# oleg-savchenko/jax_nbody_emulator_with_dj

Hardware: AMD Instinct MI355X
Metric: voxels/sec (disp+vel) on 512^3 box, ndiv=4 (higher is better)
Workload: dtype f32-equivalent: f16x3 split MFMA (3 f16 MFMAs per product, f32 accumulate)

## Files before the change

### jax_nbody_emulator_with_dj_amd/csrc/nbe_engine.cpp

```cpp

#include "../../include/nbe.h"
#include "nbe_kernels.h"

#include <sched.h>

#include <cmath>
#include <cstdarg>
#include <cstdio>
#include <cstdlib>
#include <cstring>
#include <algorithm>
#include <atomic>
#include <chrono>
#include <condition_variable>
#include <deque>
#include <map>
#include <memory>
#include <mutex>
#include <string>
#include <thread>
#include <vector>

using namespace nbe;

// ... 70 lines not shown

struct ProfEntry { std::string name; double ms = 0; int64_t launches = 0; double flops = 0; };

struct Progress {
    struct Item { hipEvent_t ev; int done, total; };
    nbe_progress_cb cb; void* user; int device;
    std::thread th; std::mutex mu; std::condition_variable cv; std::deque<Item> q; bool stop = false;
    Progress(nbe_progress_cb cb_, void* user_, int dev) : cb(cb_), user(user_), device(dev) {
        th = std::thread([this] {
            (void)hipSetDevice(device);
            for (;;) {
                Item it;
                {
                    std::unique_lock<std::mutex> lk(mu);
                    cv.wait(lk, [this] { return stop || !q.empty(); });
                    if (q.empty()) return;
                    it = q.front(); q.pop_front();
                }
                (void)hipEventSynchronize(it.ev);
                (void)hipEventDestroy(it.ev);
                cb(it.done, it.total, user);
            }
        });
    }
    void post(hipStream_t s, int done, int total) {
        hipEvent_t ev;
        if (hipEventCreateWithFlags(&ev, hipEventDisableTiming) != hipSuccess) return;
        (void)hipEventRecord(ev, s);
        { std::lock_guard<std::mutex> lk(mu); q.push_back({ev, done, total}); }
        cv.notify_one();
    }
    ~Progress() {
        { std::lock_guard<std::mutex> lk(mu); stop = true; }
        cv.notify_one();
        if (th.joinable()) th.join();
    }
};

struct nbe_ctx {
    int device = 0;
    hipStream_t own_stream = nullptr, stream = nullptr;
    int in_chan = 3, out_chan = 3, mid = 64;
    float eps = 1e-8f;
    bool vel = true;
    bool have_weights = false, style = false, modulated = false;
    float mod_Om = NAN, mod_Dz = NAN;
    std::map<std::string, Layer> layers;
    Arena arena;
    char* ws = nullptr;
    int64_t ws_bytes = 0;
    bool dry = false;
    int slab = 0;
    int slab_forced = -1;
    bool pyx = false;
    bool pyx_allowed = true;
    bool pz = false;
    bool zx = false;
    int phase = 0;
    struct BrickIO { void *send_lo = nullptr, *send_hi = nullptr; const void *recv_lo = nullptr, *recv_hi = nullptr;
                     void *skip_send_lo = nullptr, *skip_send_hi = nullptr; const void *skip_recv_lo = nullptr, *skip_recv_hi = nullptr;
                     hipEvent_t skip_ready = nullptr; } bio;
    struct StreamState {
        bool valid = false;
        int stage = 0;
        Tensor skip0, td, tin, t, h, y1, cat1, t2;
        int D = 0, H = 0, W = 0, S = 0;
        std::vector<Arena::Blk> blks; int64_t high = 0;
        float Dz = 0.f, vel_fac = 0.f, act_scale = 1.f; const char* ws = nullptr;
    } sst;
    nbe_progress_cb prog_cb = nullptr; void* prog_user = nullptr; int prog_k = 0, prog_n = 1;
    Progress* prog = nullptr;
    int max_tile = 512;
    int prec = PREC_F32;
    bool gauge = false;
    bool gauge_active = false;
    bool fuse = false;
    bool novel_fuse = false;
    int64_t bp_size[3] = {0, 0, 0}; int bp_slab = 0; int64_t bp_need = 0;
    int plan_tiles = 0;
    double plan_short_gb = 0.0;
    int64_t plan_logged = 0;
    int* gauge_flag = nullptr;
    int* wino_flag = nullptr; bool wino_ok = false;
    float act_scale = 1.f;
    float bias_scale = 1.f;
    bool bias_dirty = true;
    float bias_max = 0.f;
    float preset_absmax = -1.f;
    bool input_finite = true;
    bool range_pending = false;
    unsigned* flags = nullptr;
    float* box_in = nullptr; int64_t box_in_bytes = 0;
    char* box_out = nullptr; int64_t box_out_bytes = 0;
    struct HostPipe {
        bool active = false, out_async = false;
        bool tiles = false;
        bool slabwise = false;
        int o1 = 0, o2 = 0;
        const float* hbox = nullptr;
        bool in_pinned = false;
        int C = 0, S0 = 0, S1 = 0, S2 = 0, o0 = 0;
        std::vector<char> up;
        int gz = 0;
        char *hdisp = nullptr, *hvel = nullptr;
        char *ddisp = nullptr, *dvel = nullptr;
        int esz = 4, O0 = 0, O1 = 0, O2 = 0;
        int nstage = 0;
    } pipe;
    bool last_piped = false;
    hipStream_t up_stream = nullptr, down_stream = nullptr;
    static constexpr int NSTAGE = 3;
    char* stage_buf[NSTAGE] = {nullptr, nullptr, nullptr}; int64_t stage_bytes = 0;
    hipEvent_t stage_free[NSTAGE] = {nullptr, nullptr, nullptr};
    hipEvent_t ev_up = nullptr, ev_down = nullptr;
    struct GraphKey {
        const void *box, *disp, *velo, *ws;
        int geo[18]; float f[3]; int epoch, flags;
        bool operator<(const GraphKey& o) const { return memcmp(this, &o, sizeof *this) < 0; }
    };
    struct GraphVal { hipGraphExec_t exec = nullptr; hipGraph_t graph = nullptr; int seen = 0; uint64_t used = 0; };
    std::map<GraphKey, GraphVal> graphs;
    uint64_t graph_clock = 0, graph_replays = 0;
    int epoch = 0;
    hipEvent_t ev_g0 = nullptr, ev_g1 = nullptr;
    struct Probe {
        bool on = false, tile = false;
        int p[3] = {0, 0, 0}, nout = 0;
        int o[3] = {0, 0, 0};
        struct Slot { std::string name; int C, n, nw, level; int64_t off; };
        std::vector<Slot> slots;
        unsigned* bits = nullptr; int64_t words = 0;
        unsigned* count = nullptr;
    } probe;
    bool prof = false;
    std::vector<ProfEntry> prof_entries;
    struct Pending { int entry; hipEvent_t a, b; };
    std::vector<Pending> pending;
    std::vector<hipEvent_t> ev_pool;
};

static double hyp2f1_series(double a, double b, double c, double z) {
    double term = 1.0, sum = 1.0;
    for (int n = 0; n < 200000; ++n) {
        term *= (a + n) * (b + n) / ((c + n) * (n + 1.0)) * z;
        sum += term;
        if (std::fabs(term) < 1e-17 * std::fabs(sum)) break;
    }
    return sum;
}
static double hyp2f1(double a, double b, double c, double x) {
    if (x < 0) return std::pow(1.0 - x, -a) * hyp2f1_series(a, c - b, c, x / (x - 1.0));
    return hyp2f1_series(a, b, c, x);
}
static const double A2 = 1.0, B2 = 1.0 / 3.0, C2 = 11.0 / 6.0;

extern "C" double nbe_growth_factor(double z, double Om) {
    const double a = 1.0 / (1.0 + z), OL = 1.0 - Om;
    return a * hyp2f1(A2, B2, C2, -OL * a * a * a / Om) / hyp2f1(A2, B2, C2, -OL / Om);
}
static double growth_rate(double z, double Om) {
    const double a = 1.0 / (1.0 + z), x = -(1.0 - Om) * a * a * a / Om;
    const double F = hyp2f1(A2, B2, C2, x);
    const double dF = (A2 * B2 / C2) * hyp2f1(A2 + 1, B2 + 1, C2 + 1, x);
    return 1.0 + 3.0 * x * dF / F;
}
extern "C" double nbe_vel_norm(double z, double Om) {
// ... 106 lines not shown
    if (p.dx) p.dx += sh;
    return p;
}
static void fill_halo(nbe_ctx* c, const Tensor& t) {
    if (t.pad > 0 && !c->dry) launch_fill_yx(t.p, t.pad, c->vel, c->stream);
}
static void tfree(nbe_ctx* c, Tensor& t) { if (t.off >= 0) c->arena.release(t.off); t.off = -1; }
static Tensor zview(const Tensor& t, int z0, int nz) {
    Tensor v = t;
    v.off = -1;
    const int64_t sh = (int64_t)z0 * t.p.H * t.p.W * 4;
    if (v.p.x) v.p.x += sh;
    if (v.p.dx) v.p.dx += sh;
    v.p.D = nz;
    v.org[0] += z0;
    return v;
}
static void org_conv(const Tensor& x, int nconv, int out[3]) {
    const int p = x.pad ? nconv : 0;
    out[0] = x.org[0]; out[1] = x.org[1] - p; out[2] = x.org[2] - p;
}
static void set_org(Tensor& t, int z, int y, int x) { t.org[0] = z; t.org[1] = y; t.org[2] = x; }

static void probe_act(nbe_ctx* c, const Layer& L, const Planes& out, int g0, const int org[3], int ez, int ey, int ex, bool periodic,
                      const int* zr = nullptr) {
    auto& P = c->probe;
    if (!P.on || !P.tile || c->dry) return;
    const std::string name = L.block + "/" + L.layer;
    for (size_t i = 0; i < P.slots.size(); ++i) {
        const auto& S = P.slots[i];
        if (S.name != name) continue;
        ProbeLaunch a;
        a.x = out.x; a.pstride = out.pstride; a.H = out.H; a.W = out.W; a.g0 = g0; a.prec = c->prec; a.C = S.C;
        a.ext[0] = ez; a.ext[1] = ey; a.ext[2] = ex;
        a.org[0] = org[0]; a.org[1] = org[1]; a.org[2] = org[2];
        a.per[0] = 0; a.per[1] = periodic ? ey : 0; a.per[2] = periodic ? ex : 0;
        a.zlo = zr ? zr[0] : 0; a.zhi = zr ? zr[1] : 0; a.zper = zr ? zr[2] : 0;
        for (int d = 0; d < 3; ++d) a.o[d] = P.o[d] >> S.level;
        a.n = S.n; a.nw = S.nw;
        if (a.zper <= 0 && (a.o[0] + S.n <= org[0] || a.o[0] >= org[0] + ez)) return;
        a.bits = P.bits + S.off; a.count = P.count + i;
        launch_probe_signs(a, c->stream);
        return;
    }
}

static int prof_entry(nbe_ctx* c, const std::string& name) {
    for (size_t i = 0; i < c->prof_entries.size(); ++i) if (c->prof_entries[i].name == name) return (int)i;
    c->prof_entries.push_back({name, 0, 0, 0});
    return (int)c->prof_entries.size() - 1;
}
static hipEvent_t get_event(nbe_ctx* c) {
    if (!c->ev_pool.empty()) { hipEvent_t e = c->ev_pool.back(); c->ev_pool.pop_back(); return e; }
    hipEvent_t e; (void)hipEventCreate(&e); return e;
}
static void prof_collect(nbe_ctx* c) {
    if (c->pending.empty()) return;
    (void)hipStreamSynchronize(c->stream);
    for (auto& p : c->pending) {
        float ms = 0;
        (void)hipEventElapsedTime(&ms, p.a, p.b);
        c->prof_entries[p.entry].ms += ms;
        c->ev_pool.push_back(p.a); c->ev_pool.push_back(p.b);
    }
    c->pending.clear();
}

static std::string conv_name(const PackedW& pw, bool vel, bool has_dx, bool g6 = false, bool up8 = false) {
    if (up8) return vel ? "up_h3<8 parities,vel,dx>" : "up_h3<8 parities,novel>";
    const char* m = pw.mode == MODE_FLAT3 ? "FLAT3" : pw.mode == MODE_FLAT1 ? "FLAT1" : "DOWN";
    if (pw.stem && !(vel && has_dx) && pw.mode == MODE_FLAT3) return vel ? "stem_h3<FLAT3,vel,nodx>" : "stem_h3<FLAT3,novel>";
    char b[96];
    if (g6 && prec_is_half(pw.prec)) snprintf(b, sizeof b, "%s<%s,vel,dx>", pw.prec == PREC_F16 ? "conv_h1g" : (pw.cout_t == 16 ? "conv_h3n" : "conv_h3g"), m);
    else if (g6) snprintf(b, sizeof b, "conv_mfma_g<%s,vel,dx,ni%d>", m, pw.ni);
    else if (prec_is_half(pw.prec))
        snprintf(b, sizeof b, "%s<%s,%s,%s>", pw.prec == PREC_F16 ? "conv_h1" : "conv_h3", m, vel ? "vel" : "novel", (vel && has_dx) ? "dx" : "nodx");
    else
        snprintf(b, sizeof b, "conv_mfma<%s,%s,%s,ni%d>", m, vel ? "vel" : "novel", (vel && has_dx) ? "dx" : "nodx", pw.ni);
    return b;
}

static bool wino_f16_layer(int prec, bool vel, int cin_pad) { return prec == PREC_F16 && vel && cin_pad % 32 == 0 && cin_pad / 32 <= 8; }
static bool wino_env_off() { return getenv("NBE_WINO") && atoi(getenv("NBE_WINO")) == 0; }
static bool up8_launch(const nbe_ctx* c, const Layer& L, bool has_dx) { return prec_is_half(c->prec) && (!c->vel || has_dx) && L.pw.cin_pad <= 64; }

static int run_conv(nbe_ctx* c, const Layer& L, const ConvLaunch& cl_in, bool has_dx) {
    if (c->dry) return 0;
    ConvLaunch cl = cl_in;
    const bool g6 = c->gauge_active && L.g6 && has_dx;
    const bool nov = !c->vel && c->prec == PREC_F16X3 && L.kind == 0 && L.pw.ww && c->wino_ok;
    if (c->gauge_active) { cl.gout = L.gout; cl.beta = g6 ? L.beta : nullptr; }
    if (cl.skw) {
        if (!((g6 || nov) && c->fuse && L.fskip)) return fail("internal error: fused skip requested for %s/%s", L.block.c_str(), L.layer.c_str());
        cl.bias = L.bias_f;
    }
    const PackedW& pw = (g6 && L.kind == 0 && L.pwn.w) ? L.pwn : L.pw;
    cl.wino = (g6 || nov) && c->wino_ok && &pw == &L.pw && pw.ww && (!cl.skw || cl.skw->ww) && (c->prec == PREC_F16 || !(cl.flags & F_RES)) &&
              (cl.Dv & 1) == 0 && cl.in_off == 0 && cl.osz == 1 && !wino_env_off();
    int pe = -1; hipEvent_t ea = nullptr, eb = nullptr;
    if (c->prof) {
        std::string pn = cl.wino ? std::string(c->prec == PREC_F16 ? "conv_h1w<FLAT3,vel,dx>" : c->vel ? "conv_h3w<FLAT3,vel,dx>" : "conv_h3w<FLAT3,novel>")
                                 : conv_name(pw, c->vel, has_dx, g6, cl.set < 0);
        static const bool per_layer = getenv("NBE_PROF_LAYERS") && atoi(getenv("NBE_PROF_LAYERS")) == 1;
        if (per_layer) pn += " " + L.block + "/" + L.layer;
        pe = prof_entry(c, pn);
        ea = get_event(c); eb = get_event(c);
        (void)hipEventRecord(ea, c->stream);
    }
    if (launch_conv(pw, cl, c->vel, has_dx, c->stream))
        return fail("internal error: no kernel for layer %s/%s (mode %d, gauged %d, input tangent %d, crop offset %ld, output stride %d)",
                    L.block.c_str(), L.layer.c_str(), L.pw.mode, (int)g6, (int)has_dx, (long)cl.in_off, cl.osz);
    if (c->prof) {
        (void)hipEventRecord(eb, c->stream);
        c->pending.push_back({pe, ea, eb});
        const double nout = (double)cl.Dv * cl.Hv * cl.Wv * (cl.set < 0 ? 8.0 : 1.0);
        const int taps = L.kind == 0 ? 27 : L.kind == 2 ? 8 : 1;
        const double gemms = c->vel ? ((has_dx && !g6) ? 3.0 : 2.0) : 1.0;
        c->prof_entries[pe].flops += 2.0 * nout * L.cout * L.cin * taps * gemms;
        if (cl.skw) c->prof_entries[pe].flops += 2.0 * nout * L.cout * L.fskip->cin * (!c->vel ? 1.0 : (cl.flags & F_SKIP_NODX) ? 2.0 : 3.0);
        c->prof_entries[pe].launches += 1;
        if (c->pending.size() > 4096) prof_collect(c);
    }
    return 0;
}

static const Layer* find_layer(nbe_ctx* c, const char* block, const char* layer) {
    auto it = c->layers.find(std::string(block) + "/" + layer);
    return it == c->layers.end() ? nullptr : &it->second;
}


static bool wino_only_fuse(const nbe_ctx* c) { return !c->vel || c->prec == PREC_F16; }
static bool block_fused(const nbe_ctx* c, const Layer* L1, int nres) {
    return c->fuse && L1->fskip != nullptr && (!wino_only_fuse(c) || (!wino_env_off() && (nres & 1) == 0));
}

static Tensor alloc_hidden(nbe_ctx* c, int cmid, int nz, const Tensor& x, bool fused) {
    const int pad = x.pad, sy = pad ? 0 : 2;
    if (fused && !pad) return talloc(c, cmid, nz, x.p.H, x.p.W);
    return tallocp(c, cmid, nz, x.p.H - 2 * pad - sy, x.p.W - 2 * pad - sy, pad);
}

static int resblock_part(nbe_ctx* c, const char* name, const Tensor& x, const Tensor& h, const Tensor& s,
                         int js, int ns, int jh, int nh, bool has_dx, bool final_act, const int* zr, const Tensor* x2 = nullptr) {
    const Layer *Ls = find_layer(c, name, "skip"), *L0 = find_layer(c, name, "conv_0"), *L1 = find_layer(c, name, "conv_1");
    if (!Ls || !L0 || !L1) return fail("missing layers of block %s", name);
    const int H = x.p.H, W = x.p.W, pad = x.pad;
    const bool fused = block_fused(c, L1, ns);
    if (fused && (h.p.H != H || h.p.W != W)) return fail("internal: hidden tensor of fused block %s lacks the input's pitch", name);
    if (x2 && (!fused || x2->p.H != H || x2->p.W != W || x2->pad != pad)) return fail("internal: two-source input of block %s", name);
    const Tensor sv = zview(s, js, ns), hv = zview(h, jh, nh);
    const Tensor xs = zview(x, js, ns + 4);
    const int64_t sk_off = (2L * H + (pad ? pad : 2)) * W + (pad ? pad : 2);
    if (!fused) {
        ConvLaunch cl; cl.in = xs.p; cl.in_off = sk_off;
        cl.Dv = ns; cl.Hv = s.p.H - 2 * pad; cl.Wv = s.p.W - 2 * pad; cl.out = inner(sv); cl.flags = 0;
        if (run_conv(c, *Ls, cl, has_dx)) return 1;
    }
    int og[3];
    {
        ConvLaunch cl; cl.in = zview(x, jh, nh + 2).p; cl.Dv = nh; cl.Hv = H - 2; cl.Wv = W - 2; cl.out = inner(hv); cl.flags = F_ACT;
        if (x2) { cl.in2 = zview(*x2, jh, nh + 2).p; cl.csplit_ch = c->mid; }
        if (run_conv(c, *L0, cl, has_dx)) return 1;
        org_conv(x, 1, og); og[0] += jh;
        const int zh[3] = {zr ? zr[0] : 0, zr ? zr[1] + 2 : 0, zr ? zr[2] : 0};
        probe_act(c, *L0, cl.out, 0, og, cl.Dv, cl.Hv, cl.Wv, pad != 0, zr ? zh : nullptr);
    }
    fill_halo(c, hv);
    {
        ConvLaunch cl; cl.in = zview(h, js, ns + 2).p; cl.Dv = ns; cl.Hv = s.p.H - 2 * pad; cl.Wv = s.p.W - 2 * pad; cl.out = inner(sv);
        if (fused) { cl.sk = xs.p; cl.sk_off = sk_off; cl.skw = L1->pwn.w ? &Ls->pwn : &Ls->pw; cl.flags = (final_act ? F_ACT : 0) | (has_dx ? 0 : F_SKIP_NODX);
                     if (x2) { cl.sk2 = zview(*x2, js, ns + 4).p; cl.sk_split_ch = c->mid; } }
        else { cl.res = inner(sv); cl.flags = F_RES | (final_act ? F_ACT : 0); }
        if (run_conv(c, *L1, cl, true)) return 1;
        org_conv(x, 2, og); og[0] += js;
        if (final_act) probe_act(c, *L1, cl.out, 0, og, cl.Dv, cl.Hv, cl.Wv, pad != 0, zr);
    }
    fill_halo(c, sv);
    return 0;
}

static int resblock(nbe_ctx* c, const char* name, const Tensor& x, bool has_dx, bool final_act, int cout, int cmid, Tensor* out) {
    const Layer* L1 = find_layer(c, name, "conv_1");
    if (!L1) return fail("missing layers of block %s", name);
    const int D = x.p.D, pad = x.pad;
    const int sy = pad ? 0 : 2;
    Tensor s = tallocp(c, cout, D - 4, x.p.H - 2 * pad - 2 * sy, x.p.W - 2 * pad - 2 * sy, pad);
    Tensor h = alloc_hidden(c, cmid, D - 2, x, block_fused(c, L1, D - 4));
    if (s.off < 0 || h.off < 0) return fail("workspace exhausted in block %s", name);
    if (resblock_part(c, name, x, h, s, 0, D - 4, 0, D - 2, has_dx, final_act, nullptr)) return 1;
    tfree(c, h);
    int og[3];
    org_conv(x, 2, og);
    set_org(s, og[0], og[1], og[2]);
    *out = s;
    return 0;
}

static void carry_planes(nbe_ctx* c, const Tensor& t, int src, int dst, int n) {
    if (c->dry || n <= 0) return;
    launch_crop(zview(t, src, n).p, 0, zview(t, dst, n).p, 0, c->vel, c->stream, 0);
}

static int down_conv(nbe_ctx* c, const Layer& L, const Tensor& x, Tensor& o, bool probe) {
    ConvLaunch cl; cl.in = inner(x); cl.Dv = o.p.D; cl.Hv = o.p.H; cl.Wv = o.p.W; cl.out = o.p; cl.flags = F_ACT;
    if (run_conv(c, L, cl, true)) return 1;
    set_org(o, x.org[0] / 2, x.org[1] / 2, x.org[2] / 2);
    if (probe) probe_act(c, L, cl.out, 0, o.org, cl.Dv, cl.Hv, cl.Wv, x.pad != 0);
    return 0;
}

static int downblock(nbe_ctx* c, const char* name, const Tensor& x, Tensor* out) {
    const Layer* L = find_layer(c, name, "conv_0");
    if (!L) return fail("missing layer %s/conv_0", name);
    Tensor o = talloc(c, c->mid, x.p.D / 2, x.p.H / 2, x.p.W / 2);
    if (o.off < 0) return fail("workspace exhausted in %s", name);
    if (down_conv(c, *L, x, o, true)) return 1;
    *out = o;
    return 0;
}

static int mid_planes(const nbe_ctx* c) { return c->mid / (c->prec == PREC_F16 ? 8 : 4); }

static int upblock(nbe_ctx* c, const char* name, const Tensor& x, const Tensor& cat, int xcrop = 0, int g0 = -1) {
    const Layer* L = find_layer(c, name, "conv_0");
    if (!L) return fail("missing layer %s/conv_0", name);
    xcrop += x.pad;
    const int Hx = x.p.H - 2 * xcrop, Wx = x.p.W - 2 * xcrop;
    if (cat.p.D != 2 * x.p.D || cat.p.H - 2 * cat.pad != 2 * Hx || cat.p.W - 2 * cat.pad != 2 * Wx)
        return fail("internal: concat geometry mismatch in %s", name);
    const bool up8 = up8_launch(c, *L, true);
    const int out_g0 = g0 >= 0 ? g0 : mid_planes(c);
    for (int p = 0; p < (up8 ? 1 : 8); ++p) {
        ConvLaunch cl; cl.in = x.p; cl.in_off = ((int64_t)xcrop * x.p.W + xcrop);
        cl.Dv = x.p.D; cl.Hv = Hx; cl.Wv = Wx; cl.out = inner(cat);
        cl.out_g0 = out_g0; cl.osz = 2; cl.oz = (p >> 2) & 1; cl.oy = (p >> 1) & 1; cl.ox = p & 1;
        cl.flags = F_ACT; cl.set = up8 ? -1 : p;
        if (run_conv(c, *L, cl, true)) return 1;
    }
    const int xc = xcrop - x.pad;
    const int og[3] = {2 * x.org[0], 2 * (x.org[1] + xc), 2 * (x.org[2] + xc)};
    probe_act(c, *L, inner(cat), out_g0, og, 2 * x.p.D, 2 * Hx, 2 * Wx, cat.pad != 0);
    return 0;
}

static void crop_into(nbe_ctx* c, const Tensor& src, int crop, const Tensor& dst, int cz = -1) {
    if (c->dry) return;
    Planes s = src.p; s.G = mid_planes(c);
    launch_crop(s, crop, dst.p, 0, c->vel, c->stream, cz);
}

static int check_dims(int D, int H, int W) {
    const int v[3] = {D, H, W};
    for (int i = 0; i < 3; ++i)
        if (v[i] < 104 || v[i] % 8 != 0)
            return fail("input spatial size %d unsupported: each of (D,H,W) must be >= 104 and a multiple of 8 "
                        "(all-VALID U-Net with three 2x levels, receptive-field crop 48)", v[i]);
    return 0;
}

struct HeadOut { void* disp; void* velo; int out_dtype; int OD, OH, OW, a0, a1, a2; float Dz, vel_fac; };

static void run_head(nbe_ctx* c, const Tensor& y, const Tensor& xin, const HeadOut& h, int zoff) {
    if (c->dry) return;
    const float inv_s = 1.0f / c->act_scale;
    HeadScale hs;
    hs.k_disp = 6.0f * inv_s; hs.k_dy = h.vel_fac * 6.0f * inv_s; hs.k_x0 = h.vel_fac * 6.0f / h.Dz * inv_s;
    hs.bad = c->flags ? (int*)(c->flags + 1) : nullptr;
    launch_head(y.p, xin.p, 48, c->out_chan, hs, c->vel, h.disp, h.velo, h.out_dtype, h.OD, h.OH, h.OW,
                h.a0 + zoff, h.a1, h.a2, c->prec, c->stream, y.pad);
}

static int prepare_range(nbe_ctx* c, const float* dev_src, int64_t n, float Dz, const float* host_src = nullptr) {
// ... 210 lines not shown
static int stream_level1(nbe_ctx* c, int pad, bool pz, Tensor td, Tensor* cat1_out, Tensor* t_out) {
    const int m = c->mid;
    Tensor t = td;
    if (pad) {
        t = tallocp(c, m, td.p.D + (pz ? 44 : 0), td.p.H, td.p.W, 1);
        if (t.off < 0) return fail("workspace exhausted (level 1 input)");
        if (!c->dry) launch_wrap_pad(td.p, t.p, 1, c->vel, c->stream, pz ? 22 : 0);
        set_org(t, pz ? td.org[0] - 22 : td.org[0], td.org[1], td.org[2]);
        tfree(c, td);
    }

    Tensor y1, cat1;
    if (resblock(c, "conv_l1", t, true, true, m, m, &y1)) return 1;
    tfree(c, t);
    if (pad) {
        cat1 = tallocp(c, 2 * m, y1.p.D - 32, y1.p.H - 2, y1.p.W - 2, 1);
        if (cat1.off < 0) return fail("workspace exhausted (cat1)");
        crop_into(c, y1, 0, cat1, 16);
        set_org(cat1, y1.org[0], y1.org[1] - 16, y1.org[2] - 16);
        Tensor t2 = talloc(c, m, y1.p.D / 2, (y1.p.H - 2) / 2, (y1.p.W - 2) / 2);
        const Layer* Ld1 = find_layer(c, "down_l1", "conv_0");
        if (t2.off < 0 || !Ld1) return fail("workspace exhausted or missing layer (down_l1)");
        if (down_conv(c, *Ld1, y1, t2, true)) return 1;
        t = talloc(c, m, t2.p.D, t2.p.H + 20, t2.p.W + 20);
        if (t.off < 0) return fail("workspace exhausted (level 2 input)");
        if (!c->dry) launch_wrap_pad(t2.p, t.p, 10, c->vel, c->stream, 0);
        set_org(t, t2.org[0], t2.org[1] - 10, t2.org[2] - 10);
        tfree(c, t2);
    } else {
        cat1 = talloc(c, 2 * m, y1.p.D - 32, y1.p.H - 32, y1.p.W - 32);
        if (cat1.off < 0) return fail("workspace exhausted (cat1)");
        crop_into(c, y1, 16, cat1);
        if (downblock(c, "down_l1", y1, &t)) return 1;
    }
    tfree(c, y1);
    *cat1_out = cat1; *t_out = t;
    return 0;
}

static int lower_levels(nbe_ctx* c, Tensor t, Tensor cat1, Tensor* r_out) {
    const int m = c->mid;
    Tensor y2, cat2, r;
    if (resblock(c, "conv_l2", t, true, true, m, m, &y2)) return 1;
    tfree(c, t);
    cat2 = talloc(c, 2 * m, y2.p.D - 8, y2.p.H - 8, y2.p.W - 8);
    if (cat2.off < 0) return fail("workspace exhausted (cat2)");
    crop_into(c, y2, 4, cat2);
    if (downblock(c, "down_l2", y2, &t)) return 1;
    tfree(c, y2);

    if (resblock(c, "conv_c", t, true, true, m, m, &r)) return 1;
    tfree(c, t);

    if (upblock(c, "up_r2", r, cat2)) return 1;
    tfree(c, r);
    if (resblock(c, "conv_r2", cat2, true, true, m, 2 * m, &r)) return 1;
    tfree(c, cat2);

    if (upblock(c, "up_r1", r, cat1, cat1.pad ? 2 : 0)) return 1;
    fill_halo(c, cat1);
    tfree(c, r);
    if (resblock(c, "conv_r1", cat1, true, true, m, 2 * m, r_out)) return 1;
    tfree(c, cat1);
    return 0;
}

static int network(nbe_ctx* c, const Tensor& tin, Tensor* yout) {
    const int m = c->mid;
    Tensor a, y0, t, cat0, cat1, r;
    if (resblock(c, "conv_l00", tin, false, true, m, m, &a)) return 1;
    if (resblock(c, "conv_l01", a, true, true, m, m, &y0)) return 1;
    tfree(c, a);
    cat0 = talloc(c, 2 * m, y0.p.D - 80, y0.p.H - 80, y0.p.W - 80);
    if (cat0.off < 0) return fail("workspace exhausted (cat0)");
    crop_into(c, y0, 40, cat0);
    if (downblock(c, "down_l0", y0, &t)) return 1;
    tfree(c, y0);

    if (stream_level1(c, 0, false, t, &cat1, &t)) return 1;
    if (lower_levels(c, t, cat1, &r)) return 1;

    if (upblock(c, "up_r0", r, cat0)) return 1;
    tfree(c, r);
    if (resblock(c, "conv_r00", cat0, true, true, m, 2 * m, &r)) return 1;
    tfree(c, cat0);

    if (resblock(c, "conv_r01", r, true, false, c->out_chan, m, yout)) return 1;
    tfree(c, r);
    return 0;
}

static constexpr int BRICK_H1 = 6, BRICK_H2 = 10;
static constexpr int BRICK_H0 = 4;
static Planes brick_planes(nbe_ctx* c, const Tensor& like, const void* buf, int nplanes) {
    Planes p = like.p;
    p.D = nplanes;
    p.pstride = (p.vox() + 63) & ~int64_t(63);
    p.x = (float*)buf;
    p.dx = c->vel ? (float*)buf + (int64_t)p.G * p.pstride * 4 : nullptr;
    return p;
}
static void brick_send(nbe_ctx* c, const Tensor& t, int in, int n, void* lo, void* hi) {
    if (c->dry) return;
    for (int s = 0; s < 2; ++s)
        launch_crop(zview(t, s ? t.p.D - in - n : in, n).p, 0, brick_planes(c, t, s ? hi : lo, n), 0, c->vel, c->stream, 0);
}
static void brick_recv(nbe_ctx* c, const Tensor& like, const void* lo, const void* hi, int n, const Tensor& dst, int wrap) {
    if (c->dry) return;
    for (int s = 0; s < 2; ++s) {
        const Planes face = brick_planes(c, like, s ? hi : lo, n), to = zview(dst, s ? dst.p.D - n : 0, n).p;
        if (wrap) launch_wrap_pad(face, to, wrap, c->vel, c->stream, 0);
        else launch_crop(face, 0, to, 0, c->vel, c->stream, 0);
    }
}
static int64_t brick_halo_bytes(nbe_ctx* c, int nplanes, int Hd, int Wd) {
    Planes p; p.G = planes_for(c->mid, c->prec); p.D = nplanes; p.H = Hd; p.W = Wd;
    p.pstride = (p.vox() + 63) & ~int64_t(63);
    return (int64_t)p.G * p.pstride * 16 * (c->vel ? 2 : 1);
}

static int brick_conv_l1(nbe_ctx* c, const Tensor& t, const Tensor& h, const Tensor& y1, int part) {
    const int B = t.p.D - 2 * BRICK_H1;
    if (part == 0) return resblock_part(c, "conv_l1", t, h, y1, BRICK_H1, B - 4, BRICK_H1, B - 2, true, true, nullptr);
    if (part == 1) return resblock_part(c, "conv_l1", t, h, y1, 0, BRICK_H1, 0, BRICK_H1, true, true, nullptr);
    return resblock_part(c, "conv_l1", t, h, y1, B + 2, BRICK_H1, B + 4, BRICK_H1, true, true, nullptr);
}

static int brick_interior(nbe_ctx* c, nbe_ctx::StreamState& st) {
    const int m = c->mid;
    const Tensor& td = st.td;
    const Layer* L1 = find_layer(c, "conv_l1", "conv_1");
    if (!L1) return fail("missing layer conv_l1/conv_1");
    st.t = tallocp(c, m, td.p.D + 2 * BRICK_H1, td.p.H, td.p.W, 1);
    if (st.t.off < 0) return fail("workspace exhausted (level 1 input)");
    st.h = alloc_hidden(c, m, st.t.p.D - 2, st.t, block_fused(c, L1, st.t.p.D - 4));
    st.y1 = tallocp(c, m, st.t.p.D - 4, td.p.H, td.p.W, 1);
    if (st.h.off < 0 || st.y1.off < 0) return fail("workspace exhausted (level 1)");
    if (!c->dry) launch_wrap_pad(td.p, zview(st.t, BRICK_H1, td.p.D).p, 1, c->vel, c->stream, 0);
    return brick_conv_l1(c, st.t, st.h, st.y1, 0);
}

static int brick_edges(nbe_ctx* c, nbe_ctx::StreamState& st) {
    const int m = c->mid;
    Tensor& td = st.td;
    const int B = td.p.D;
    brick_recv(c, td, c->bio.recv_lo, c->bio.recv_hi, BRICK_H1, st.t, 1);
    if (brick_conv_l1(c, st.t, st.h, st.y1, 1) || brick_conv_l1(c, st.t, st.h, st.y1, 2)) return 1;
    tfree(c, st.h); tfree(c, st.t); tfree(c, td);
    Tensor& y1 = st.y1;
    st.cat1 = tallocp(c, 2 * m, y1.p.D, y1.p.H - 2, y1.p.W - 2, 1);
    if (st.cat1.off < 0) return fail("workspace exhausted (cat1)");
    crop_into(c, y1, 0, st.cat1, 0);
    st.t2 = talloc(c, m, B / 2, (y1.p.H - 2) / 2, (y1.p.W - 2) / 2);
    const Layer* Ld1 = find_layer(c, "down_l1", "conv_0");
    if (st.t2.off < 0 || !Ld1) return fail("workspace exhausted or missing layer (down_l1)");
    if (down_conv(c, *Ld1, zview(y1, 4, B), st.t2, false)) return 1;
    tfree(c, y1);
    if (c->bio.send_lo) brick_send(c, st.t2, 0, BRICK_H2, c->bio.send_lo, c->bio.send_hi);
    return 0;
}

static int brick_level2(nbe_ctx* c, nbe_ctx::StreamState& st, Tensor* t_out) {
    Tensor& t2 = st.t2;
    Tensor t = talloc(c, c->mid, t2.p.D + 2 * BRICK_H2, t2.p.H + 20, t2.p.W + 20);
    if (t.off < 0) return fail("workspace exhausted (level 2 input)");
    if (!c->dry) launch_wrap_pad(t2.p, zview(t, BRICK_H2, t2.p.D).p, 10, c->vel, c->stream, 0);
    brick_recv(c, t2, c->bio.recv_lo, c->bio.recv_hi, BRICK_H2, t, 10);
    tfree(c, t2);
    *t_out = t;
    return 0;
}

static int stream_tail(nbe_ctx* c, const Tensor& tin, const HeadOut& ho, int S, Tensor skip0, Tensor cat1, Tensor t) {
    const int m = c->mid, pad = tin.pad;
    const int sy = pad ? 0 : 2;
    const Layer *Lr00 = find_layer(c, "conv_r00", "conv_1"), *Lr01 = find_layer(c, "conv_r01", "conv_1");
    if (!Lr00 || !Lr01) return fail("missing conv_1 layers of the level-0 blocks");
    Tensor r;
    if (lower_levels(c, t, cat1, &r)) return 1;
    if (2 * r.p.D != skip0.p.D || 2 * (r.p.H - 2 * r.pad) != skip0.p.H - 2 * pad || 2 * (r.p.W - 2 * r.pad) != skip0.p.W - 2 * pad)
        return fail("internal: level-0 concat geometry mismatch");

    if (pad && c->zx && !c->dry && c->bio.skip_recv_lo) {
        if (c->bio.skip_ready) HIPCHK(hipStreamWaitEvent(c->stream, c->bio.skip_ready, 0));
        brick_recv(c, skip0, c->bio.skip_recv_lo, c->bio.skip_recv_hi, BRICK_H0, skip0, 0);
    }
    const int Yo = skip0.p.D - 8;
    const int Hs = skip0.p.H - 2 * pad, Ws = skip0.p.W - 2 * pad;
    const bool two = block_fused(c, Lr00, S + 4) && c->mid % 16 == 0;
    Tensor cat = tallocp(c, two ? m : 2 * m, S + 8, Hs, Ws, pad), hq = alloc_hidden(c, 2 * m, S + 6, cat, block_fused(c, Lr00, S + 4));
    Tensor q = tallocp(c, m, S + 4, Hs - 2 * sy, Ws - 2 * sy, pad), hy = alloc_hidden(c, m, S + 2, q, block_fused(c, Lr01, S));
    Tensor y = tallocp(c, c->out_chan, S, Hs - 4 * sy, Ws - 4 * sy, pad);
    if (cat.off < 0 || hq.off < 0 || q.off < 0 || hy.off < 0 || y.off < 0) return fail("workspace exhausted (level-0 decoder slabs)");
    for (int z = 0, n = 0; z < Yo; z += n) {
        n = std::min(S, Yo - z);
        if (c->pipe.active && c->pipe.out_async && Yo - z > PIPE_EDGE && Yo - z - n < PIPE_EDGE)
            n = Yo - z - PIPE_EDGE;
        const bool first = z == 0;
        const int c0 = first ? 0 : 8, cn = first ? n + 8 : n;
        set_org(cat, skip0.org[0] + z, skip0.org[1], skip0.org[2]);
        { int og[3]; org_conv(cat, 2, og); set_org(q, og[0], og[1], og[2]); }
        if (!two && !c->dry) launch_crop(zview(skip0, z + c0, cn).p, 0, zview(cat, c0, cn).p, 0, c->vel, c->stream, 0);
        if (upblock(c, "up_r0", zview(r, (z + c0) / 2, cn / 2), zview(cat, c0, cn), 0, two ? 0 : -1)) return 1;
        fill_halo(c, zview(cat, c0, cn));
        const Tensor sk = two ? zview(skip0, z, std::min(S + 8, skip0.p.D - z)) : cat;
        const Tensor* up2 = two ? &cat : nullptr;
        if (first) {
            if (resblock_part(c, "conv_r00", sk, hq, q, 0, n + 4, 0, n + 6, true, true, nullptr, up2)) return 1;
            if (resblock_part(c, "conv_r01", q, hy, y, 0, n, 0, n + 2, true, false, nullptr)) return 1;
        } else {
            if (resblock_part(c, "conv_r00", sk, hq, q, 4, n, 6, n, true, true, nullptr, up2)) return 1;
            if (resblock_part(c, "conv_r01", q, hy, y, 0, n, 2, n, true, false, nullptr)) return 1;
        }
        if (z + n < Yo) {
            carry_planes(c, cat, n, 0, 8);
            carry_planes(c, hq, n, 0, 6);
            carry_planes(c, q, n, 0, 4);
            carry_planes(c, hy, n, 0, 2);
        }
        run_head(c, zview(y, 0, n), zview(tin, z, n + 96), ho, z);
        if (c->pipe.active && c->pipe.out_async && !c->dry && pipe_output(c, z, n)) return 1;
        if (c->prog && !c->dry && z + n < Yo)
            c->prog->post(c->pipe.active && c->pipe.out_async ? c->down_stream : c->stream,
                          c->prog_k * 1000 + (int)(1000L * (z + n) / Yo), c->prog_n * 1000);
    }
    tfree(c, cat); tfree(c, hq); tfree(c, q); tfree(c, hy); tfree(c, y);
    tfree(c, r); tfree(c, skip0);
    return 0;
}

static void stash_arena(nbe_ctx* c) { c->sst.blks = c->arena.blks; c->sst.high = c->arena.high; }

static int network_stream(nbe_ctx* c, const Tensor& tin, const HeadOut& ho, int S) {
    auto& st = c->sst;
    const int pad = tin.pad;
    const bool zx = pad && c->zx;
    if (c->phase >= 2) {
        if (!st.valid || st.stage != c->phase - 1) return fail("brick calls out of order (encode, interior, exchange, finish) or the context was used in between");
        c->arena.blks = st.blks; c->arena.high = st.high;
    }
    if (c->phase <= 1) {
        if (stream_encode(c, tin, ho, S, &st.skip0, &st.td)) return 1;
        st.tin = tin; st.S = S;
        if (c->phase == 1) {
            brick_send(c, st.td, 0, BRICK_H1, c->bio.send_lo, c->bio.send_hi);
            brick_send(c, st.skip0, BRICK_H0, BRICK_H0, c->bio.skip_send_lo, c->bio.skip_send_hi);
            st.valid = true; st.stage = 1; stash_arena(c);
            return 0;
        }
    }
    if (!zx) {
        Tensor cat1, t;
        if (stream_level1(c, pad, pad && c->pz, st.td, &cat1, &t)) return 1;
        return stream_tail(c, tin, ho, S, st.skip0, cat1, t);
    }
    if (c->phase == 0 || c->phase == 2) {
        if (brick_interior(c, st)) return 1;
        if (c->phase == 2) { st.stage = 2; stash_arena(c); return 0; }
    }
    if (c->phase == 0 || c->phase == 3) {
        if (brick_edges(c, st)) return 1;
        if (c->phase == 3) { st.stage = 3; stash_arena(c); return 0; }
    }
    Tensor t;
    if (brick_level2(c, st, &t)) return 1;
    st.valid = false;
    return stream_tail(c, st.tin, ho, st.S, st.skip0, st.cat1, t);
}

static int check_dims_pyx(int D, int H, int W) {
    if (D < 104 || D % 8 != 0) return fail("input depth %d unsupported: must be >= 104 and a multiple of 8", D);
    const int v[2] = {H - 2, W - 2};
    for (int i = 0; i < 2; ++i)
        if (v[i] < 48 || v[i] % 8 != 0) return fail("periodic extent %d unsupported: must be >= 48 and a multiple of 8", v[i]);
    return 0;
}

static int64_t workspace_need(nbe_ctx* c, int D, int H, int W, int slab, bool pyx, bool pz) {
    const int keep_slab = c->slab; const bool keep_pyx = c->pyx, keep_pz = c->pz;
    c->slab = slab; c->pyx = pyx; c->pz = pz;
    c->dry = true;
    c->arena.reset();
    Tensor tin = talloc(c, c->in_chan, D, H, W), y;
    tin.pad = c->pyx ? 1 : 0;
    HeadOut ho{};
    const int rc = c->slab > 0 ? network_stream(c, tin, ho, c->slab) : network(c, tin, &y);
    c->dry = false;
    c->slab = keep_slab; c->pyx = keep_pyx; c->pz = keep_pz;
    return rc ? -1 : c->arena.high;
}

static int ensure_workspace(nbe_ctx* c, int D, int H, int W) {
    const int64_t need = workspace_need(c, D, H, W, c->slab, c->pyx, c->pz);
    if (need < 0) return 1;
    if (need > c->ws_bytes) {
        c->sst.valid = false;
        if (c->ws) { HIPCHK(hipStreamSynchronize(c->stream)); HIPCHK(hipFree(c->ws)); c->ws = nullptr; c->ws_bytes = 0; }
        HIPCHK(hipMalloc((void**)&c->ws, need));
        HIPCHK(hipMemsetAsync(c->ws, 0, need, c->stream));
        c->ws_bytes = need;
    }
    return 0;
}

static int require_ready(nbe_ctx* c) {
    if (!c->have_weights) return fail("No parameters loaded. Call nbe_load_style_weights / nbe_load_premod_weights first.");
    if (c->style && !c->modulated) return fail("style weights are loaded but nbe_set_cosmology(Om, Dz) has not been called");
    return 0;
}

static int run_subbox(nbe_ctx* c, const float* box, int Db, int Hb, int Wb, int o0, int o1, int o2,
                      int D, int H, int W, float Dz, float vel_fac, void* disp, void* velo, int out_dtype,
                      int OD, int OH, int OW, int a0, int a1, int a2) {
    c->sst.valid = false;
    c->arena.reset();
    Tensor tin = talloc(c, c->in_chan, D, H, W), y;
    tin.pad = c->pyx ? 1 : 0;
    if (tin.pad) set_org(tin, 0, 48, 48);
    if (!c->pipe.active && !c->pipe.slabwise)
        launch_gather(box, c->in_chan, Db, Hb, Wb, o0, o1, o2, tin.p, Dz / 6.0f * c->act_scale, c->prec, c->stream);
    const HeadOut ho{disp, velo, out_dtype, OD, OH, OW, a0, a1, a2, Dz, vel_fac};
    if (c->slab > 0) return network_stream(c, tin, ho, c->slab);
    if (network(c, tin, &y)) return 1;
    run_head(c, y, tin, ho, 0);
    return 0;
}

static void drop_graphs(nbe_ctx* c) {
    for (auto& kv : c->graphs) {
        if (kv.second.exec) (void)hipGraphExecDestroy(kv.second.exec);
        if (kv.second.graph) (void)hipGraphDestroy(kv.second.graph);
    }
    c->graphs.clear();
}

static int run_tile(nbe_ctx* c, const float* box, int Db, int Hb, int Wb, int o0, int o1, int o2,
                    int D, int H, int W, float Dz, float vel_fac, void* disp, void* velo, int out_dtype,
                    int OD, int OH, int OW, int a0, int a1, int a2) {
    const bool off = getenv("NBE_GRAPH") && atoi(getenv("NBE_GRAPH")) == 0;
    if (off || c->prof || c->prog_cb || c->pipe.active || c->pipe.slabwise || c->dry || c->probe.on)
        return run_subbox(c, box, Db, Hb, Wb, o0, o1, o2, D, H, W, Dz, vel_fac, disp, velo, out_dtype, OD, OH, OW, a0, a1, a2);
    nbe_ctx::GraphKey k;
    memset(&k, 0, sizeof k);
    k.box = box; k.disp = disp; k.velo = velo; k.ws = c->ws;
    const int geo[18] = {Db, Hb, Wb, o0, o1, o2, D, H, W, out_dtype, OD, OH, OW, a0, a1, a2, c->slab, c->prec};
    memcpy(k.geo, geo, sizeof geo);
    k.f[0] = Dz; k.f[1] = vel_fac; k.f[2] = c->act_scale;
    k.epoch = c->epoch; k.flags = (c->pyx ? 1 : 0) | (c->pz ? 2 : 0) | (c->gauge_active ? 4 : 0) | (c->fuse ? 8 : 0) | (wino_env_off() ? 16 : 0);
    nbe_ctx::GraphVal& g = c->graphs[k];
    g.used = ++c->graph_clock;
    if (!g.exec && g.seen++ == 0) {
        if (c->graphs.size() > 16) {
            auto lru = c->graphs.begin();
            for (auto it = c->graphs.begin(); it != c->graphs.end(); ++it) if (it->second.used < lru->second.used) lru = it;
            if (lru->second.exec) (void)hipGraphExecDestroy(lru->second.exec);
            if (lru->second.graph) (void)hipGraphDestroy(lru->second.graph);
            c->graphs.erase(lru);
        }
        return run_subbox(c, box, Db, Hb, Wb, o0, o1, o2, D, H, W, Dz, vel_fac, disp, velo, out_dtype, OD, OH, OW, a0, a1, a2);
    }
    if (!c->ev_g0) { HIPCHK(hipEventCreateWithFlags(&c->ev_g0, hipEventDisableTiming)); HIPCHK(hipEventCreateWithFlags(&c->ev_g1, hipEventDisableTiming)); }
    hipStream_t user = c->stream;
    if (!g.exec) {
        c->stream = c->own_stream;
        hipError_t e = hipStreamBeginCapture(c->own_stream, hipStreamCaptureModeThreadLocal);
        int rc = 0;
        if (e == hipSuccess) {
            rc = run_subbox(c, box, Db, Hb, Wb, o0, o1, o2, D, H, W, Dz, vel_fac, disp, velo, out_dtype, OD, OH, OW, a0, a1, a2);
            e = hipStreamEndCapture(c->own_stream, &g.graph);
            if (e == hipSuccess && !rc) e = hipGraphInstantiate(&g.exec, g.graph, nullptr, nullptr, 0);
        }
        c->stream = user;
        if (rc || e != hipSuccess || !g.exec) {
            (void)hipGetLastError();
            if (g.graph) { (void)hipGraphDestroy(g.graph); g.graph = nullptr; }
            g.exec = nullptr; g.seen = -1000000;
            return run_subbox(c, box, Db, Hb, Wb, o0, o1, o2, D, H, W, Dz, vel_fac, disp, velo, out_dtype, OD, OH, OW, a0, a1, a2);
        }
    }
    if (user != c->own_stream) { HIPCHK(hipEventRecord(c->ev_g0, user)); HIPCHK(hipStreamWaitEvent(c->own_stream, c->ev_g0, 0)); }
    HIPCHK(hipGraphLaunch(g.exec, c->own_stream));
    if (user != c->own_stream) { HIPCHK(hipEventRecord(c->ev_g1, c->own_stream)); HIPCHK(hipStreamWaitEvent(user, c->ev_g1, 0)); }
    ++c->graph_replays;
    return 0;
}

static void free_layers(nbe_ctx* c) {
    drop_graphs(c); ++c->epoch;
    for (auto& kv : c->layers) {
        Layer& L = kv.second;
        (void)hipFree(L.weight); (void)hipFree(L.sw); (void)hipFree(L.sb); (void)hipFree(L.wn); (void)hipFree(L.dwn);
        (void)hipFree(L.pw.w); (void)hipFree(L.pw.dw); (void)hipFree(L.pw.bias); (void)hipFree(L.bias0); (void)hipFree(L.pw.stem); (void)hipFree(L.pw.ww); (void)hipFree(L.pwn.w); (void)hipFree(L.pwn.dw); (void)hipFree(L.bias_f);
        (void)hipFree(L.alpha); (void)hipFree(L.beta); (void)hipFree(L.dwn_f);
    }
    c->layers.clear();
    c->bias_scale = 1.f; c->bias_max = 0.f; c->bias_dirty = true;
    c->have_weights = false; c->modulated = false; c->gauge = false; c->gauge_active = false; c->fuse = false; c->novel_fuse = false; c->wino_ok = false;
}

static int kind_of(const nbe_layer_desc& d, int* kind) {
    const std::string blk = d.block, lay = d.layer;
    if (lay == "skip") { if (d.k != 1) return fail("%s/%s: skip layers have k=1", d.block, d.layer); *kind = 1; return 0; }
    if (blk.rfind("down_", 0) == 0) { if (d.k != 2) return fail("%s: down layers have k=2", d.block); *kind = 2; return 0; }
    if (blk.rfind("up_", 0) == 0) { if (d.k != 2) return fail("%s: up layers have k=2", d.block); *kind = 3; return 0; }
    if (d.k != 3) return fail("%s/%s: conv layers have k=3", d.block, d.layer);
    *kind = 0;
    return 0;
}

static int expected_shape(nbe_ctx* c, const std::string& blk, const std::string& lay, int* cout, int* cin) {
    const int m = c->mid;
    int bi, bo;
    if (blk == "conv_l00") { bi = c->in_chan; bo = m; }
    else if (blk == "conv_r2" || blk == "conv_r1" || blk == "conv_r00") { bi = 2 * m; bo = m; }
    else if (blk == "conv_r01") { bi = m; bo = c->out_chan; }
    else { bi = m; bo = m; }
    const int midc = bi > bo ? bi : bo;
    if (lay == "skip") { *cin = bi; *cout = bo; }
    else if (blk.rfind("down_", 0) == 0 || blk.rfind("up_", 0) == 0) { *cin = bi; *cout = bo; }
    else if (lay == "conv_0") { *cin = bi; *cout = midc; }
    else if (lay == "conv_1") { *cin = midc; *cout = bo; }
    else return fail("unknown layer %s/%s", blk.c_str(), lay.c_str());
    return 0;
}

static const char* kBlocks[15] = {"conv_l00", "conv_l01", "down_l0", "conv_l1", "down_l1", "conv_l2", "down_l2", "conv_c",
                                  "up_r2", "conv_r2", "up_r1", "conv_r1", "up_r0", "conv_r00", "conv_r01"};

static int pack_wino(nbe_ctx* c) {
    c->wino_ok = false;
    if (!((c->prec == PREC_F16X3 && (c->vel ? c->gauge_active : true)) || (c->prec == PREC_F16 && c->vel && c->gauge_active))) return 0;
    if (!c->wino_flag) HIPCHK(hipMalloc((void**)&c->wino_flag, 4));
    HIPCHK(hipMemsetAsync(c->wino_flag, 0, 4, c->stream));
    for (auto& kv : c->layers) {
        Layer& L = kv.second;
        if (L.pw.ww && L.kind == 0 && (L.g6 || !c->vel)) launch_pack_h3w(L.wn, L.cout, L.cin, L.pw.cin_pad, L.pw.ctiles, L.pw.ww, c->wino_flag, c->stream, c->prec);
        if (L.pw.ww && L.kind == 1 && (c->vel ? (L.b_sub && c->fuse) : c->novel_fuse)) {
            launch_pack_h3w_skip(L.wn, L.cout, L.cin, L.pw, L.pw.ww, c->wino_flag, c->stream);
            if (c->vel) launch_pack_h3w_skip(c->prec == PREC_F16 ? L.dwn_f : L.dwn, L.cout, L.cin, L.pw, L.pw.ww + L.pw.floats, c->wino_flag, c->stream);
        }
    }
    int bad = 0;
    HIPCHK(hipMemcpyAsync(&bad, c->wino_flag, 4, hipMemcpyDeviceToHost, c->stream));
    HIPCHK(hipStreamSynchronize(c->stream));
    c->wino_ok = bad == 0;
    if (!c->vel) c->fuse = c->novel_fuse && c->wino_ok;
    if (c->prec == PREC_F16) c->fuse = c->fuse && c->wino_ok;
    return 0;
}

static int wire_novel(nbe_ctx* c) {
    c->novel_fuse = false;
    if (c->vel || c->prec != PREC_F16X3) return 0;
    for (const char* b : kBlocks) {
        if (!strncmp(b, "down_", 5) || !strncmp(b, "up_", 3)) continue;
        auto i1 = c->layers.find(std::string(b) + "/conv_1"), is = c->layers.find(std::string(b) + "/skip");
        if (i1 == c->layers.end() || is == c->layers.end()) return fail("internal: block %s", b);
        Layer &L1 = i1->second, &Ls = is->second;
        if (!L1.pw.ww || !Ls.pw.ww || 2 * (Ls.pw.cin_pad / 16) > 16 || L1.pw.ctiles != Ls.pw.ctiles) return 0;
    }
    for (const char* b : kBlocks) {
        if (!strncmp(b, "down_", 5) || !strncmp(b, "up_", 3)) continue;
        Layer &L1 = c->layers[std::string(b) + "/conv_1"], &Ls = c->layers[std::string(b) + "/skip"];
        L1.fskip = &Ls;
        const int nb = L1.pw.ctiles * 32 * L1.pw.ni;
        HIPCHK(hipMalloc((void**)&L1.bias_f, nb * 4));
    }
    c->novel_fuse = true;
    return 0;
}

static int wire_gauge(nbe_ctx* c) {
    const int m = c->mid;
    for (auto& kv : c->layers) {
        Layer& L = kv.second;
        const size_t na = (size_t)roundup(L.cin, 16) + 64, nb = (size_t)L.pw.ctiles * 32 * L.pw.ni + 64;
        HIPCHK(hipMalloc((void**)&L.alpha, na * 4)); HIPCHK(hipMemset(L.alpha, 0, na * 4));
        HIPCHK(hipMalloc((void**)&L.beta, nb * 4)); HIPCHK(hipMemset(L.beta, 0, nb * 4));
    }
    if (!c->gauge_flag) HIPCHK(hipMalloc((void**)&c->gauge_flag, 4));
    auto lay = [&](const char* b, const char* l) -> Layer* {
        auto it = c->layers.find(std::string(b) + "/" + l);
        return it == c->layers.end() ? nullptr : &it->second;
    };
    struct Rule { const char* pb; const char* pl; const char* consumer; int off; };
    const Rule rules[] = {
        {"conv_l00", "conv_1", "conv_l01", 0}, {"conv_l01", "conv_1", "conv_r00", 0}, {"down_l0", "conv_0", "conv_l1", 0},
        {"conv_l1", "conv_1", "conv_r1", 0},   {"down_l1", "conv_0", "conv_l2", 0},   {"conv_l2", "conv_1", "conv_r2", 0},
        {"down_l2", "conv_0", "conv_c", 0},    {"up_r2", "conv_0", "conv_r2", m},     {"up_r1", "conv_0", "conv_r1", m},
        {"up_r0", "conv_0", "conv_r00", m},    {"conv_r00", "conv_1", "conv_r01", 0},
    };
    for (const Rule& r : rules) {
        Layer *P = lay(r.pb, r.pl), *C = lay(r.consumer, "conv_0");
        if (!P || !C || r.off + P->cout > C->cin) return fail("internal: gauge wiring %s/%s -> %s", r.pb, r.pl, r.consumer);
        P->gout = C->alpha + r.off;
    }
    for (const char* b : kBlocks) {
        if (!strncmp(b, "down_", 5) || !strncmp(b, "up_", 3)) continue;
        Layer *L0 = lay(b, "conv_0"), *L1 = lay(b, "conv_1"), *Ls = lay(b, "skip");
        L0->gout = L1->alpha;
        L1->g6 = true;
        if (strcmp(b, "conv_l00")) { L0->g6 = true; Ls->a_in = L0->alpha; }
        if (c->prec == PREC_F16X3 && (!L1->pwn.w || Ls->pwn.dw) &&
            3 * (L1->pw.cin_pad / 16) + Ls->pw.cin_pad / 16 <= NBE_MAX_GROUPS) {
            L1->fskip = Ls; Ls->b_sub = L1->beta;
            const int nb = L1->pw.ctiles * 32 * L1->pw.ni;
            HIPCHK(hipMalloc((void**)&L1->bias_f, nb * 4));
        }
        if (c->prec == PREC_F16 && L1->pw.ww && Ls->pw.ww && Ls->dwn_f && L1->pw.ctiles == Ls->pw.ctiles &&
            2 * (Ls->pw.cin_pad / 32) <= 16) {
            L1->fskip = Ls; Ls->b_sub = L1->beta;
            const int nb = L1->pw.ctiles * 32 * L1->pw.ni;
            HIPCHK(hipMalloc((void**)&L1->bias_f, nb * 4));
        }
    }
    for (auto& kv : c->layers)
        if (kv.second.g6 && 3 * (kv.second.pw.cin_pad / 16) > NBE_MAX_GROUPS) { c->gauge = false; return 0; }
    lay("down_l0", "conv_0")->a_in = lay("conv_r00", "conv_0")->alpha;
    lay("down_l1", "conv_0")->a_in = lay("conv_r1", "conv_0")->alpha;
    lay("down_l2", "conv_0")->a_in = lay("conv_r2", "conv_0")->alpha;
    c->gauge = true;
    return 0;
}

static int wire_gauge_premod(nbe_ctx* c, const nbe_layer_desc* descs, int n) {
    std::map<std::string, std::vector<double>> al, be;
    std::map<std::string, const nbe_layer_desc*> by_name;
    for (int i = 0; i < n; ++i) by_name[std::string(descs[i].block) + "/" + descs[i].layer] = &descs[i];
// ... 140 lines not shown
        if (style && L.kind == 1 && !L.first && wino_f16_layer(c->prec, c->vel, pw.cin_pad)) {
            HIPCHK(hipMalloc((void**)&pw.ww, pw.floats * 2 * 4));
            HIPCHK(hipMalloc((void**)&L.dwn_f, nw * 4));
        }
        if (prec_is_half(c->prec) && L.kind == 0 && L.first && d.cin <= 3 && d.cout <= 64)
            HIPCHK(hipMalloc((void**)&pw.stem, 4 * 3 * 4 * 64 * 16));
        HIPCHK(hipMalloc((void**)&L.bias0, nb * 4));
        HIPCHK(hipMemcpy(L.bias0, pw.bias, nb * 4, hipMemcpyDeviceToDevice));
        for (int i = 0; i < d.cout; ++i)
            if (std::isfinite(d.bias[i])) c->bias_max = std::max(c->bias_max, std::fabs(d.bias[i]));
        HIPCHK(hipMalloc((void**)&L.wn, nw * 4));
        if (c->vel) HIPCHK(hipMalloc((void**)&L.dwn, nw * 4));
        if (style) {
            if (!d.style_weight || !d.style_bias) return fail("%s/%s: style_weight and style_bias are required", d.block, d.layer);
            HIPCHK(hipMalloc((void**)&L.weight, nw * 4));
            HIPCHK(hipMalloc((void**)&L.sw, d.cin * 2 * 4));
            HIPCHK(hipMalloc((void**)&L.sb, d.cin * 4));
            HIPCHK(hipMemcpy(L.weight, d.weight, nw * 4, hipMemcpyHostToDevice));
            HIPCHK(hipMemcpy(L.sw, d.style_weight, d.cin * 2 * 4, hipMemcpyHostToDevice));
            HIPCHK(hipMemcpy(L.sb, d.style_bias, d.cin * 4, hipMemcpyHostToDevice));
        } else {
            if (c->vel && !d.dweight) return fail("%s/%s: dweight is required for premodulated velocity weights", d.block, d.layer);
            HIPCHK(hipMemcpy(L.wn, d.weight, nw * 4, hipMemcpyHostToDevice));
            if (c->vel) HIPCHK(hipMemcpy(L.dwn, d.dweight, nw * 4, hipMemcpyHostToDevice));
            launch_pack(L.wn, d.cout, d.cin, L.kind, pw, pw.w, c->stream);
            if (c->vel) launch_pack(L.dwn, d.cout, d.cin, L.kind, pw, pw.dw, c->stream);
            if (L.pwn.w) launch_pack(L.wn, d.cout, d.cin, L.kind, L.pwn, L.pwn.w, c->stream);
            if (L.pwn.dw) launch_pack(L.dwn, d.cout, d.cin, L.kind, L.pwn, L.pwn.dw, c->stream);
        }
        c->layers[L.block + "/" + L.layer] = L;
    }
    for (const char* b : kBlocks) {
        const bool rs = !strncmp(b, "down_", 5) || !strncmp(b, "up_", 3);
        const char* need[3] = {"conv_0", rs ? nullptr : "skip", rs ? nullptr : "conv_1"};
        for (const char* l : need)
            if (l && !find_layer(c, b, l)) return fail("parameter tree is missing %s/%s", b, l);
    }
    HIPCHK(hipStreamSynchronize(c->stream));
    c->have_weights = true; c->style = style; c->modulated = !style;
    c->mod_Om = NAN; c->mod_Dz = NAN;
    const char* ge = getenv("NBE_GAUGE");
    if (c->vel && !(ge && atoi(ge) == 0)) return style ? wire_gauge(c) : wire_gauge_premod(c, descs, n);
    if (!c->vel) {
        if (wire_novel(c)) return 1;
        if (!style) return pack_wino(c);
    }
    return 0;
}

extern "C" {

const char* nbe_last_error(void) { return g_err.c_str(); }
int nbe_version(void) { return 100; }

int nbe_create(int device_id, nbe_ctx** out) {
    if (!out) return fail("nbe_create: out is NULL");
    int ndev = 0;
    if (hipGetDeviceCount(&ndev) != hipSuccess || ndev == 0)
        return fail("nbe_create: no HIP device is visible; this library has no CPU fallback");
    if (device_id < 0 || device_id >= ndev) return fail("nbe_create: device %d out of range (0..%d)", device_id, ndev - 1);
    HIPCHK(hipSetDevice(device_id));
    hipDeviceProp_t prop;
    HIPCHK(hipGetDeviceProperties(&prop, device_id));
    if (!strstr(prop.gcnArchName, "gfx950"))
        return fail("nbe_create: device %d is %s; the kernels are built for gfx950 (MI355X) only", device_id, prop.gcnArchName);
    nbe_ctx* c = new nbe_ctx();
    c->device = device_id;
    HIPCHK(hipStreamCreateWithFlags(&c->own_stream, hipStreamNonBlocking));
    c->stream = c->own_stream;
    if (const char* e = getenv("NBE_MAX_TILE")) c->max_tile = atoi(e) > 0 ? atoi(e) : 0;
    if (const char* e = getenv("NBE_SLAB")) c->slab_forced = atoi(e) >= 0 ? (atoi(e) & ~1) : -1;
    if (const char* e = getenv("NBE_PERIODIC")) c->pyx_allowed = atoi(e) != 0;
    *out = c;
    return 0;
}

int nbe_destroy(nbe_ctx* c) {
    if (!c) return 0;
    (void)hipSetDevice(c->device);
    (void)hipStreamSynchronize(c->stream);
    prof_collect(c);
    free_layers(c);
    (void)hipFree(c->probe.bits); (void)hipFree(c->probe.count);
    (void)hipFree(c->ws); (void)hipFree(c->box_in); (void)hipFree(c->box_out); (void)hipFree(c->gauge_flag); (void)hipFree(c->wino_flag); (void)hipFree(c->flags);
    drop_graphs(c);
    if (c->ev_g0) (void)hipEventDestroy(c->ev_g0);
    if (c->ev_g1) (void)hipEventDestroy(c->ev_g1);
    for (auto e : c->ev_pool) (void)hipEventDestroy(e);
    for (int i = 0; i < nbe_ctx::NSTAGE; ++i) { if (c->stage_buf[i]) (void)hipHostFree(c->stage_buf[i]); if (c->stage_free[i]) (void)hipEventDestroy(c->stage_free[i]); }
    if (c->ev_up) (void)hipEventDestroy(c->ev_up);
    if (c->ev_down) (void)hipEventDestroy(c->ev_down);
    if (c->up_stream) (void)hipStreamDestroy(c->up_stream);
    if (c->down_stream) (void)hipStreamDestroy(c->down_stream);
    (void)hipStreamDestroy(c->own_stream);
    delete c;
    return 0;
}

int nbe_set_stream(nbe_ctx* c, void* s) {
    if (!c) return fail("null context");
    HIPCHK(hipStreamSynchronize(c->stream));
    c->stream = (hipStream_t)s;
    return 0;
}

int nbe_use_own_stream(nbe_ctx* c) {
    if (!c) return fail("null context");
    HIPCHK(hipStreamSynchronize(c->stream));
    c->stream = c->own_stream;
    return 0;
}

int nbe_synchronize(nbe_ctx* c) {
    if (!c) return fail("null context");
    HIPCHK(hipStreamSynchronize(c->stream));
    return 0;
}

int nbe_set_arch(nbe_ctx* c, int in_chan, int out_chan, int mid_chan, float eps, int compute_vel) {
    if (!c) return fail("null context");
    if (in_chan < 1 || in_chan > 16) return fail("in_chan=%d unsupported (1..16)", in_chan);
    if (out_chan < 1 || out_chan > 64) return fail("out_chan=%d unsupported (1..64)", out_chan);
    if (out_chan != in_chan) return fail("out_chan (%d) must equal in_chan (%d): the head adds the cropped input (core :187)", out_chan, in_chan);
    if (mid_chan < 8 || mid_chan % 8 != 0) return fail("mid_chan=%d unsupported (multiple of 8 required)", mid_chan);
    HIPCHK(hipSetDevice(c->device));
    HIPCHK(hipStreamSynchronize(c->stream));
    free_layers(c);
    c->in_chan = in_chan; c->out_chan = out_chan; c->mid = mid_chan; c->eps = eps; c->vel = compute_vel != 0;
    return 0;
}

int nbe_load_style_weights(nbe_ctx* c, const nbe_layer_desc* layers, int n) {
    if (!c || !layers) return fail("null argument");
    return load_weights(c, layers, n, true);
}

int nbe_load_premod_weights(nbe_ctx* c, const nbe_layer_desc* layers, int n) {
    if (!c || !layers) return fail("null argument");
    return load_weights(c, layers, n, false);
}

int nbe_set_cosmology(nbe_ctx* c, float Om, float Dz) {
    if (!c) return fail("null context");
    if (!c->have_weights) return fail("No parameters loaded. Call nbe_load_style_weights first.");
    if (!c->style) return 0;
    if (c->modulated && c->mod_Om == Om && c->mod_Dz == Dz) return 0;
    c->sst.valid = false;
    HIPCHK(hipSetDevice(c->device));
    const float s0 = (Om - 0.3f) * 5.0f, s1 = Dz - 1.0f;
    bool use_gauge = c->gauge;
    if (use_gauge) {
        HIPCHK(hipMemsetAsync(c->gauge_flag, 0, 4, c->stream));
        for (auto& kv : c->layers)
            launch_style_alpha(kv.second.sw, kv.second.sb, kv.second.cin, s0, s1, kv.second.alpha, c->gauge_flag, c->stream);
        int bad = 0;
        HIPCHK(hipMemcpyAsync(&bad, c->gauge_flag, 4, hipMemcpyDeviceToHost, c->stream));
        HIPCHK(hipStreamSynchronize(c->stream));
        use_gauge = bad == 0;
    }
    for (auto& kv : c->layers) {
        Layer& L = kv.second;
        launch_modulate(L.weight, L.sw, L.sb, L.cout, L.cin, L.k * L.k * L.k, s0, s1, c->eps, L.first ? 1 : 0,
                        L.wn, c->vel ? L.dwn : nullptr, c->stream, use_gauge ? L.a_in : nullptr, use_gauge ? L.beta : nullptr,
                        (use_gauge && c->prec != PREC_F16) ? L.b_sub : nullptr);
        if (use_gauge && c->prec == PREC_F16 && c->vel && L.b_sub && L.dwn_f)
            launch_modulate(L.weight, L.sw, L.sb, L.cout, L.cin, L.k * L.k * L.k, s0, s1, c->eps, L.first ? 1 : 0,
                            L.wn, L.dwn_f, c->stream, L.a_in, nullptr, L.b_sub);
// ... 912 lines not shown
```

### jax_nbody_emulator_with_dj_amd/csrc/nbe_kernels.h

```cpp
#pragma once
#include <hip/hip_runtime.h>
#include <stdint.h>

namespace nbe {

struct Planes {
    float* x = nullptr;
    float* dx = nullptr;
    int64_t pstride = 0;
    int G = 0;
    int D = 0, H = 0, W = 0;
    int64_t vox() const { return (int64_t)D * H * W; }
};

enum Precision { PREC_F32 = 0, PREC_F16X3 = 1, PREC_F16 = 2 };
inline constexpr bool prec_is_half(int prec) { return prec == PREC_F16X3 || prec == PREC_F16; }
inline constexpr int prec_parts(int prec) { return prec == PREC_F16X3 ? 2 : 1; }
constexpr float H3_SCALE = 2048.0f, H3_INV = 1.0f / 2048.0f;
constexpr int H3_RANGE_UP = 6;

constexpr int NBE_MAX_GROUPS = 64;

enum ConvMode { MODE_FLAT3 = 0, MODE_FLAT1 = 1, MODE_DOWN = 2 };
enum ConvFlags { F_ACT = 1, F_RES = 2, F_SKIP_NODX = 4 };

constexpr int TILE_VOX = 256;
inline constexpr int mode_taps(int mode) { return mode == MODE_FLAT3 ? 3 : 1; }
inline constexpr int mode_nseg(int mode) { return mode == MODE_FLAT3 ? 9 : (mode == MODE_DOWN ? 8 : 1); }
inline constexpr int mode_ck(int mode) { return mode == MODE_FLAT3 ? 8 : 16; }
inline constexpr int prec_ck(int prec, int mode) { return prec_is_half(prec) ? 16 : mode_ck(mode); }

struct PackedW {
    float* w = nullptr;
    float* dw = nullptr;
    float* bias = nullptr;
    int prec = PREC_F32;
    int mode = 0, ni = 2;
    int cout_t = 64;
    int cin = 0, cout = 0;
    int cin_pad = 0;
    int ctiles = 0;
    int64_t floats = 0;
    int nsets = 1;
    float* ww = nullptr;
    float* stem = nullptr;
};

struct ConvLaunch {
    Planes in;
    int64_t in_off = 0;
    int Dv = 0, Hv = 0, Wv = 0;
    Planes out;
    int out_g0 = 0;
    int osz = 1, oz = 0, oy = 0, ox = 0;
    Planes res;
    int flags = 0;
    int set = 0;
    const float* gout = nullptr;
    const float* beta = nullptr;
    const float* bias = nullptr;
    Planes in2;
    int csplit_ch = 0;
    Planes sk, sk2;
    int sk_split_ch = 0;
    int64_t sk_off = 0;
    const PackedW* skw = nullptr;
    bool wino = false;
};

int launch_conv(const PackedW& pw, const ConvLaunch& L, bool vel, bool has_dx, hipStream_t s);

void launch_modulate(const float* weight, const float* style_weight, const float* style_bias,
                     int cout, int cin, int k3, float s0, float s1, float eps, int first_layer,
                     float* w_n, float* dw_tot , hipStream_t s,
                     const float* a_in = nullptr, float* beta_out = nullptr, const float* b_sub = nullptr);
void launch_style_alpha(const float* style_weight, const float* style_bias, int cin, float s0, float s1,
                        float* alpha, int* flag, hipStream_t s);
void launch_pack(const float* w_oidhw, int cout, int cin, int kind, const PackedW& pw, float* dst, hipStream_t s);

void launch_pack_h3w(const float* w_oidhw, int cout, int cin, int cin_pad, int ctiles, float* dst, int* flag, hipStream_t s,
                     int prec = PREC_F16X3);
void launch_pack_h3w_skip(const float* w_oidhw, int cout, int cin, const PackedW& pw, float* dst, int* flag, hipStream_t s);

void launch_gather(const float* box, int C, int Db, int Hb, int Wb, int a0, int a1, int a2,
                   const Planes& dst, float scale, int prec, hipStream_t s);
void launch_to_planes(const float* src, int C, const Planes& dst, bool tangent, float scale, int prec, hipStream_t s);
void launch_from_planes(const Planes& src, bool tangent, int C, float* dst, int prec, hipStream_t s);
void launch_crop(const Planes& src, int c, const Planes& dst, int g0, bool vel, hipStream_t s, int cz = -1);
struct HeadScale { float k_disp = 6.f, k_dy = 0.f, k_x0 = 0.f; int* bad = nullptr; };
void launch_head(const Planes& y, const Planes& xin, int c0, int C, const HeadScale& hs, bool vel,
                 void* disp, void* velo, int out_dtype, int Db, int Hb, int Wb, int a0, int a1, int a2,
                 int prec, hipStream_t s, int pad = 0);
void launch_absmax(const float* src, int64_t n, unsigned* out_bits, hipStream_t s);
void launch_zero(void* dst, int64_t bytes, hipStream_t s);
void launch_scale(const float* src, float* dst, int n, float f, hipStream_t s, const float* src2 = nullptr);

void launch_fill_yx(const Planes& t, int pad, bool vel, hipStream_t s);
void launch_wrap_pad(const Planes& src, const Planes& dst, int pad, bool vel, hipStream_t s, int padz = 0);

void launch_tag_word(unsigned* dst, unsigned v, const unsigned* expect_at, unsigned* flag, unsigned bit, hipStream_t s);

struct ProbeLaunch {
    const float* x; int64_t pstride; int H, W, g0, prec, C;
    int ext[3], org[3], per[3];
    int zlo, zhi, zper;
    int o[3], n, nw;
    unsigned* bits; unsigned* count;
};
void launch_probe_signs(const ProbeLaunch& a, hipStream_t s);

void h3q_read_stamps(double* out16, hipStream_t s);

}
```

### jax_nbody_emulator_with_dj_amd/csrc/nbe_kernels.hip

```cpp

#include "nbe_kernels_internal.h"
#include <algorithm>
#include <cstdint>
#include <cstdio>
#include <cstdlib>

namespace nbe {

#define LDS_AS NBE_LDS_AS
#define GLB_AS NBE_GLB_AS

extern __shared__ __attribute__((aligned(16))) f32x4 lds_dyn[];

template <int MODE, bool VEL, bool HAS_DX, int NI, bool G6 = false>
__global__ __launch_bounds__(256, 2) void conv_mfma_kernel(ConvKArgs a) {
    constexpr int CK = mode_ck(MODE), GL = CK / 4, TAPS = mode_taps(MODE);
    constexpr int COUT_T = 32 * NI;
    constexpr int XV = (MODE == MODE_FLAT3) ? 320 : 256;
    constexpr int WP = TAPS * GL * COUT_T;
    constexpr int XP = GL * XV;
    constexpr bool DX = VEL && HAS_DX;
    constexpr bool DWT = VEL && !G6;
    static_assert(!G6 || (DX && MODE == MODE_FLAT3), "gauged form: 3x3x3 layers with an input tangent");
    constexpr int OFF_W = 0, OFF_DW = WP, OFF_X = OFF_DW + (DWT ? WP : 0), OFF_DXX = OFF_X + XP;
// ... 136 lines not shown
                if (cg >= a.cout_groups) continue;
                const f32x4 bv = *(const f32x4*)(a.bias + cg * 4);
                f32x4 v, dv;
#pragma unroll
                for (int e = 0; e < 4; ++e) { v[e] = accy[it][jt][4 * k + e] + bv[e]; dv[e] = accd[it][jt][4 * k + e]; }
                if (G6) {
                    const f32x4 be = *(const f32x4*)(a.beta + cg * 4);
#pragma unroll
                    for (int e = 0; e < 4; ++e) dv[e] += be[e] * accy[it][jt][4 * k + e];
                }
                if (res) {
                    const long ro = ((long)cg * a.res_pstride + o) * 4;
                    const f32x4 rv = *(const f32x4*)(a.r + ro);
                    v += rv;
                    if (VEL) { const f32x4 drv = *(const f32x4*)(a.dr + ro); dv += drv; }
                }
                if (act) {
#pragma unroll
                    for (int e = 0; e < 4; ++e) {
                        if (VEL) dv[e] = v[e] > 0.f ? dv[e] : 0.01f * dv[e];
                        v[e] = v[e] >= 0.f ? v[e] : 0.01f * v[e];
                    }
                }
                if (VEL && a.gout) {
                    const f32x4 gv = *(const f32x4*)(a.gout + cg * 4);
#pragma unroll
                    for (int e = 0; e < 4; ++e) dv[e] += gv[e] * v[e];
                }
                const long oo = ((long)(a.out_g0 + cg) * a.out_pstride + o) * 4;
                *(f32x4*)(a.y + oo) = v;
                if (VEL) *(f32x4*)(a.dy + oo) = dv;
            }
        }
    }
}

template <int MODE, bool VEL, bool HAS_DX, int NI, bool G6 = false>
static void launch_conv_t(const ConvKArgs& ka, int ctiles, hipStream_t s) {
    constexpr int CK = mode_ck(MODE), GL = CK / 4, TAPS = mode_taps(MODE);
    constexpr int XV = (MODE == MODE_FLAT3) ? 320 : 256;
    constexpr int WP = TAPS * GL * 32 * NI, XP = GL * XV;
    constexpr int BUF = WP * ((VEL && !G6) ? 2 : 1) + XP * ((VEL && HAS_DX) ? 2 : 1);
    constexpr size_t smem = (size_t)2 * BUF * 16 + 256 * sizeof(int);
    auto kern = conv_mfma_kernel<MODE, VEL, HAS_DX, NI, G6>;
    ensure_lds_limit((const void*)kern, smem);
    dim3 grid(ka.ntiles, ctiles, 1), block(256, 1, 1);
    hipLaunchKernelGGL(kern, grid, block, smem, s, ka);
}

int launch_conv(const PackedW& pw, const ConvLaunch& L, bool vel, bool has_dx, hipStream_t s) {
    ConvKArgs ka;
    ka.x = L.in.x; ka.dx = L.in.dx; ka.in_pstride = L.in.pstride;
    ka.D = L.in.D; ka.H = L.in.H; ka.W = L.in.W; ka.P = L.in.vox(); ka.in_off = L.in_off;
    ka.Dv = L.Dv; ka.Hv = L.Hv; ka.Wv = L.Wv;
    if (pw.mode == MODE_DOWN) ka.Q = (long)L.Dv * L.Hv * L.Wv;
    else ka.Q = ((long)(L.Dv - 1) * L.in.H + (L.Hv - 1)) * L.in.W + L.Wv;
    ka.y = L.out.x; ka.dy = L.out.dx; ka.out_pstride = L.out.pstride; ka.out_g0 = L.out_g0;
    ka.Ho = L.out.H; ka.Wo = L.out.W; ka.osz = L.osz; ka.oz = L.oz; ka.oy = L.oy; ka.ox = L.ox;
    ka.r = L.res.x; ka.dr = L.res.dx; ka.res_pstride = L.res.pstride;
    ka.bias = L.bias ? L.bias : pw.bias;
    const int set = L.set < 0 ? 0 : L.set;
    ka.up8 = L.set < 0 ? 1 : 0; ka.set_stride = (long)pw.floats * 4;
    ka.stem_w = pw.stem;
    ka.ww = L.wino ? pw.ww : nullptr;
    ka.wws = (L.wino && L.skw) ? L.skw->ww : nullptr; ka.wws_set_floats = L.skw ? L.skw->floats : 0;
    ka.w = pw.w + (size_t)set * pw.floats;
    ka.dw = pw.dw ? pw.dw + (size_t)set * pw.floats : nullptr;
    ka.nchunk = pw.cin_pad / prec_ck(pw.prec, pw.mode);
    ka.cout_groups = prec_is_half(pw.prec) ? (pw.cout + 7) / 8 : (pw.cout + 3) / 4;
    ka.flags = L.flags;
    ka.gout = L.gout; ka.beta = L.beta;
    ka.x2 = L.in2.x; ka.dx2 = L.in2.dx; ka.in2_pstride = L.in2.pstride;
    if (L.csplit_ch % 16 != 0 || L.sk_split_ch % 16 != 0) return 1;
    ka.csplit = L.csplit_ch > 0 ? L.csplit_ch / 16 : (1 << 30);
    ka.xs = ka.dxs = ka.xs2 = ka.dxs2 = nullptr; ka.s_pstride = ka.s2_pstride = 0; ka.s_csplit = 1 << 30;
    ka.ws = ka.dws = nullptr; ka.nskip = 0; ka.dws_delta = 0;
    if (L.skw) {
        if (L.sk.H != L.in.H || L.sk.W != L.in.W) return 1;
        const int64_t o = (L.sk_off - L.sk.W - 1) * 4;
        ka.xs = L.sk.x + o; ka.dxs = (L.flags & F_SKIP_NODX) ? ka.xs : L.sk.dx + o; ka.s_pstride = L.sk.pstride;
        if (L.sk_split_ch > 0) { ka.xs2 = L.sk2.x + o; ka.dxs2 = L.sk2.dx + o; ka.s2_pstride = L.sk2.pstride; ka.s_csplit = L.sk_split_ch / 16; }
        ka.ws = L.skw->w; ka.dws = L.skw->dw; ka.nskip = L.skw->cin_pad / 16;
    }
    ka.ntiles = (int)((ka.Q + TILE_VOX - 1) / TILE_VOX);
    if (prec_is_half(pw.prec)) return launch_conv_h3(pw, ka, vel, has_dx, s);
    const int ct = pw.ctiles;
    if (ka.beta) {
        if (!(pw.mode == MODE_FLAT3 && vel && has_dx)) return 1;
        if (pw.ni == 2) launch_conv_t<MODE_FLAT3, true, true, 2, true>(ka, ct, s);
        else launch_conv_t<MODE_FLAT3, true, true, 1, true>(ka, ct, s);
        return 0;
    }
#define NBE_DISPATCH(MODE)                                                                   \
    if (vel) {                                                                               \
        if (has_dx) { if (pw.ni == 2) launch_conv_t<MODE, true, true, 2>(ka, ct, s);        \
                      else launch_conv_t<MODE, true, true, 1>(ka, ct, s); }                 \
        else        { if (pw.ni == 2) launch_conv_t<MODE, true, false, 2>(ka, ct, s);       \
                      else launch_conv_t<MODE, true, false, 1>(ka, ct, s); }                \
    } else {                                                                                 \
        if (pw.ni == 2) launch_conv_t<MODE, false, false, 2>(ka, ct, s);                     \
        else launch_conv_t<MODE, false, false, 1>(ka, ct, s);                                \
    }
    if (pw.mode == MODE_FLAT3) { NBE_DISPATCH(MODE_FLAT3) }
    else if (pw.mode == MODE_FLAT1) { NBE_DISPATCH(MODE_FLAT1) }
    else { NBE_DISPATCH(MODE_DOWN) }
#undef NBE_DISPATCH
    return 0;
}


__device__ __forceinline__ double block_sum(double v, double* scratch) {
#pragma unroll
    for (int off = 32; off > 0; off >>= 1) v += __shfl_down(v, off, 64);
    const int lane = threadIdx.x & 63, wave = threadIdx.x >> 6;
    __syncthreads();
    if (lane == 0) scratch[wave] = v;
    __syncthreads();
    double t = 0.0;
    for (int i = 0; i < (int)(blockDim.x >> 6); ++i) t += scratch[i];
    return t;
}

__global__ __launch_bounds__(256) void modulate_kernel(const float* __restrict__ weight,
                                                       const float* __restrict__ sw,
                                                       const float* __restrict__ sb,
                                                       int cin, int k3, float s0, float s1, float eps,
                                                       int first_layer, float* __restrict__ w_n,
                                                       float* __restrict__ dw_tot, const float* __restrict__ a_in,
                                                       float* __restrict__ beta_out, const float* __restrict__ b_sub) {
    __shared__ double scratch[4];
    const int co = blockIdx.x;
    const int n = cin * k3;
    const float* wr = weight + (size_t)co * n;
    double sww = 0.0, swd = 0.0;
    for (int e = threadIdx.x; e < n; e += blockDim.x) {
        const int ci = e / k3;
        const float smod = sw[2 * ci] * s0 + sw[2 * ci + 1] * s1 + sb[ci];
        const float w = wr[e] * smod;
        const float dws = wr[e] * sw[2 * ci + 1];
        sww += (double)w * w;
        swd += (double)w * dws;
    }
    sww = block_sum(sww, scratch);
    swd = block_sum(swd, scratch);
    const float norm = sqrtf((float)sww + eps);
    const float dnorm = -(float)swd / (norm * norm * norm);
    const float inv_dz = 1.0f / (s1 + 1.0f);
    if (beta_out && threadIdx.x == 0) beta_out[co] = dnorm * norm;
    for (int e = threadIdx.x; e < n; e += blockDim.x) {
        const int ci = e / k3;
        const float smod = sw[2 * ci] * s0 + sw[2 * ci + 1] * s1 + sb[ci];
        const float w = wr[e] * smod;
        const float dws = wr[e] * sw[2 * ci + 1];
        const float wn = w / norm;
        w_n[(size_t)co * n + e] = wn;
        if (dw_tot) {
            float d = dws / norm + w * dnorm;
            if (first_layer) d += wn * inv_dz;
            if (a_in) d -= wn * a_in[ci];
            if (b_sub) d -= wn * b_sub[co];
            dw_tot[(size_t)co * n + e] = d;
        }
    }
}

void launch_modulate(const float* weight, const float* style_weight, const float* style_bias,
// ... 349 lines not shown
```

### jax_nbody_emulator_with_dj_amd/csrc/nbe_kernels_h3.hip

```cpp

#include "nbe_kernels_internal.h"
#include <cstdlib>
#include <cstdio>
#include <algorithm>

#ifndef NBE_DBG
#define NBE_DBG 0
#endif

namespace nbe {

extern __shared__ __attribute__((aligned(16))) f32x4 lds_h3[];

__device__ __forceinline__ void split4(const f32x4 v, half4& hi, half4& lo) {
#pragma unroll
    for (int e = 0; e < 4; ++e) {
        hi[e] = (_Float16)v[e];
        lo[e] = (_Float16)__builtin_fmaf((float)hi[e], -H3_SCALE, v[e] * H3_SCALE);
    }
}
__device__ __forceinline__ f32x4 join4(const half4 hi, const half4 lo) {
    f32x4 v;
#pragma unroll
    for (int e = 0; e < 4; ++e) v[e] = (float)hi[e] + (float)lo[e] * H3_INV;
// ... 1692 lines not shown
            for (int nt = 0; nt < 2; ++nt) {
                const int t = 2 * mt + nt;
                f32x4 v, dv;
#pragma unroll
                for (int e = 0; e < 4; ++e) {
                    v[e] = ym[t][e] + (SPLIT ? yc[t][e] * H3_INV : 0.f) + bv[e];
                    dv[e] = dm[t][e] + (SPLIT ? dc[t][e] * H3_INV : 0.f);
                }
                if (act) {
#pragma unroll
                    for (int e = 0; e < 4; ++e) {
                        dv[e] = v[e] > 0.f ? dv[e] : 0.01f * dv[e];
                        v[e] = v[e] >= 0.f ? v[e] : 0.01f * v[e];
                    }
                }
                if (gauge) {
#pragma unroll
                    for (int e = 0; e < 4; ++e) dv[e] += gv[e] * v[e];
                }
                if (!SPLIT) {
                    if (uok && ook[nt]) {
                        const long ob = ((long)(a.out_g0 + unit) * a.out_pstride + o[nt]) * 16 + 8 * kh;
                        half4 h;
#pragma unroll
                        for (int e = 0; e < 4; ++e) h[e] = (_Float16)v[e];
                        *(half4*)((char*)a.y + ob) = h;
                        if (VEL) {
#pragma unroll
                            for (int e = 0; e < 4; ++e) h[e] = (_Float16)dv[e];
                            *(half4*)((char*)a.dy + ob) = h;
                        }
                    }
                } else
                if (uok && ook[nt]) {
                    const long ob = ((long)(a.out_g0 + 2 * unit) * a.out_pstride + o[nt]) * 16 + 8 * kh;
                    const long ol = ob + a.out_pstride * 16;
                    half4 hi, lo;
                    split4(v, hi, lo);
                    *(half4*)((char*)a.y + ob) = hi;
                    *(half4*)((char*)a.y + ol) = lo;
                    if (VEL) {
                        split4(dv, hi, lo);
                        *(half4*)((char*)a.dy + ob) = hi;
                        *(half4*)((char*)a.dy + ol) = lo;
                    }
                }
            }
        }
    }
}

template <bool VEL, bool SPLIT = true>
static int launch_stem(ConvKArgs ka, hipStream_t s) {
    ka.tny = (ka.Hv + ST_ROWS - 1) / ST_ROWS;
    ka.tnx = (ka.Wv + ST_COLS - 1) / ST_COLS;
    const long nt = (long)ka.Dv * ka.tny * ka.tnx;
    if (nt <= 0 || nt >= (1L << 31) || ka.cout_groups > 8 || ka.nchunk != 1) return 1;
    ka.ntiles = (int)nt;
    const int grid = (int)std::min<long>(nt, 512);
    static_assert(2 * ST_LDS <= 160 * 1024, "two workgroups per CU");
    ensure_lds_limit((const void*)stem_h3_kernel<VEL, SPLIT>, ST_LDS);
    hipLaunchKernelGGL((stem_h3_kernel<VEL, SPLIT>), dim3(grid), dim3(256), ST_LDS, s, ka);
    return 0;
}

__global__ __launch_bounds__(256) void pack_stem_kernel(const float* __restrict__ w, int cout, int cin, _Float16* __restrict__ dst, int parts) {
    const int idx = blockIdx.x * blockDim.x + threadIdx.x;
    if (idx >= parts * 3 * 4 * 64 * 8) return;
    const int j = idx & 7, co = (idx >> 3) & 63, qq = (idx >> 9) & 3, sp = idx >> 11, st = sp % 3, part = sp / 3;
    const int k = 32 * st + 8 * qq + j, tap = k / 3, ch = k - 3 * tap;
    float v = 0.f;
    if (k < 81 && ch < cin && co < cout) v = w[((size_t)co * cin + ch) * 27 + tap];
    const _Float16 hi = (_Float16)v;
    dst[idx] = part == 0 ? hi : (_Float16)((v - (float)hi) * H3_SCALE);
}

int launch_conv_h3(const PackedW& pw, const ConvKArgs& ka, bool vel, bool has_dx, hipStream_t s) {
    const int ct = pw.ctiles;
    const bool split = pw.prec == PREC_F16X3;
    if (ka.stem_w && !(vel && has_dx) && pw.mode == MODE_FLAT3 && ka.in_off == 0 && ka.osz == 1 &&
        !(ka.flags & F_RES) && ka.nskip == 0 && !ka.beta) {
        if (split) return vel ? launch_stem<true>(ka, s) : launch_stem<false>(ka, s);
        return vel ? launch_stem<true, false>(ka, s) : launch_stem<false, false>(ka, s);
    }
    if ((ka.nskip > 0 || ka.csplit < ka.nchunk) && !(ka.beta && split)) {
        if (split && !vel && ka.ww && pw.mode == MODE_FLAT3 && ka.in_off == 0 && ka.osz == 1)
            return launch_h3w(ka, ka.ww, ka.wws, ka.wws_set_floats, ct, s, true);
        if (!split && vel && has_dx && ka.beta && ka.ww && pw.mode == MODE_FLAT3 && ka.in_off == 0 && ka.osz == 1)
            return launch_h3w(ka, ka.ww, ka.wws, ka.wws_set_floats, ct, s, false, true);
        return 1;
    }
    if (ka.beta) {
        if (!(pw.mode == MODE_FLAT3 && vel && has_dx && ka.in_off == 0 && ka.osz == 1)) return 1;
        if (split) {
            if (pw.cout_t == 16) {
                if (launch_h3n4(ka, ct, s) == 0) return 0;
                return launch_h3g<true>(ka, ct, s);
            }
            if (ka.ww && launch_h3w(ka, ka.ww, ka.wws, ka.wws_set_floats, ct, s) == 0) return 0;
            return launch_h3g<false>(ka, ct, s);
        }
        if (ka.ww && launch_h3w(ka, ka.ww, ka.wws, ka.wws_set_floats, ct, s, false, true) == 0) return 0;
        return launch_h2q<false, true>(ka, ct, s);
    }
    if (pw.mode == MODE_FLAT3) {
        if (!(ka.in_off == 0 && ka.osz == 1)) return 1;
        if (split && vel && has_dx) return launch_h3q(ka, ct, s);
        if (split && !vel && ka.ww && launch_h3w(ka, ka.ww, ka.wws, ka.wws_set_floats, ct, s, true) == 0) return 0;
        if (split && !vel) return launch_h2q<true>(ka, ct, s);
        if (!split && vel && has_dx) return launch_h2q<false>(ka, ct, s);
        if (!vel) launch_h3p_t<false, false, false>(ka, ct, s);
        else if (split) launch_h3p_t<true, false, true>(ka, ct, s);
        else launch_h3p_t<true, false, false>(ka, ct, s);
        return 0;
    }
    if (pw.mode == MODE_FLAT1) {
        if (ka.up8) {
            if (vel && has_dx) return split ? launch_up_h3<true>(ka, ct, s) : launch_up_h3<false>(ka, ct, s);
            if (!vel) return split ? launch_up_h3<true, false>(ka, ct, s) : launch_up_h3<false, false>(ka, ct, s);
            return 1;
        }
        return split ? launch_h3_vd<MODE_FLAT1, true>(ka, ct, vel, has_dx, s) : launch_h3_vd<MODE_FLAT1, false>(ka, ct, vel, has_dx, s);
    }
    return split ? launch_h3_vd<MODE_DOWN, true>(ka, ct, vel, has_dx, s) : launch_h3_vd<MODE_DOWN, false>(ka, ct, vel, has_dx, s);
}

__global__ __launch_bounds__(256) void pack_h3_kernel(const float* __restrict__ w, int cout, int cin, int kind,
                                                      int mode, int nchunk, long halves_per_set, int nsets,
                                                      int parts, int cout_t, _Float16* __restrict__ dst,
                                                      float wscale = 0.f, int* __restrict__ flag = nullptr, int f16w = 0) {
    const long idx = (long)blockIdx.x * blockDim.x + threadIdx.x;
    if (idx >= halves_per_set * nsets) return;
    const int TAPS = mode_taps(mode), nseg = mode_nseg(mode);
    const int nstage = nseg * nchunk;
    long r = idx;
    const int j = (int)(r % 8); r /= 8;
    const int co = (int)(r % cout_t); r /= cout_t;
    const int un = 2 * parts;
    const int u = (int)(r % un); r /= un;
    const int tap = (int)(r % TAPS); r /= TAPS;
    const int stage = (int)(r % nstage); r /= nstage;
    const long per_set_ct = halves_per_set / ((long)nstage * TAPS * un * cout_t * 8);
    const int ct = (int)(r % per_set_ct); r /= per_set_ct;
    const int set = (int)r;
    const int chunk = stage / nseg, seg = stage - chunk * nseg;
    const int h = u / parts, part = u - h * parts;
    const int ci = f16w ? chunk * 32 + 8 * u + j : chunk * 16 + 8 * h + j;
    const int oc = ct * cout_t + co;
    int k, kz, ky, kx;
    if (kind == 0) { k = 3; kz = seg / 3; ky = seg % 3; kx = tap; }
    else if (kind == 1) { k = 1; kz = ky = kx = 0; }
    else if (kind == 2) { k = 2; kz = seg >> 2; ky = (seg >> 1) & 1; kx = seg & 1; }
    else { k = 2; kz = 1 - ((set >> 2) & 1); ky = 1 - ((set >> 1) & 1); kx = 1 - (set & 1); }
    float v = 0.f;
    if (oc < cout && ci < cin) v = w[(((size_t)oc * cin + ci) * k + kz) * k * k + ky * k + kx];
    if (wscale != 0.f) {
        v *= wscale;
        if (!(fabsf(v) <= 60000.f)) { atomicOr(flag, 1); v = 0.f; }
        const _Float16 h = (_Float16)v;
        dst[idx] = (part == 0 || f16w) ? h : (_Float16)(v - (float)h);
        return;
    }
    const _Float16 hi = (_Float16)v;
    dst[idx] = part == 0 ? hi : (_Float16)((v - (float)hi) * H3_SCALE);
}

void launch_pack_h3w_skip(const float* w_oidhw, int cout, int cin, const PackedW& pw, float* dst, int* flag, hipStream_t s) {
    const long halves = pw.floats * 2;
    if (pw.prec == PREC_F16) {
        hipLaunchKernelGGL(pack_h3_kernel, dim3((unsigned)((halves + 255) / 256)), dim3(256), 0, s, w_oidhw, cout, cin,
                           1, pw.mode, pw.cin_pad / 32, halves, 1, 2, pw.cout_t, (_Float16*)dst, 256.0f, flag, 1);
        return;
    }
    hipLaunchKernelGGL(pack_h3_kernel, dim3((unsigned)((halves + 255) / 256)), dim3(256), 0, s, w_oidhw, cout, cin,
                       1, pw.mode, pw.cin_pad / 16, halves, 1, 2, pw.cout_t, (_Float16*)dst, 16384.0f, flag);
}

void launch_pack_h3(const float* w_oidhw, int cout, int cin, int kind, const PackedW& pw, float* dst, hipStream_t s) {
    if (pw.stem && kind == 0 && (dst == pw.w || dst == pw.dw)) {
        const int parts = pw.prec == PREC_F16X3 ? 2 : 1;
        hipLaunchKernelGGL(pack_stem_kernel, dim3(48), dim3(256), 0, s, w_oidhw, cout, cin,
                           (_Float16*)pw.stem + (dst == pw.dw ? parts * 3 * 4 * 64 * 8 : 0), parts);
    }
    const long halves = pw.floats * 2;
    const long total = halves * pw.nsets;
    hipLaunchKernelGGL(pack_h3_kernel, dim3((unsigned)((total + 255) / 256)), dim3(256), 0, s, w_oidhw, cout, cin,
                       kind, pw.mode, pw.cin_pad / 16, halves, pw.nsets, pw.prec == PREC_F16X3 ? 2 : 1, pw.cout_t,
                       (_Float16*)dst);
}

__device__ __forceinline__ half8 ld8(const float* base, long plane, long pstride, long v) {
    return *(const half8*)(base + (plane * pstride + v) * 4);
}
__device__ __forceinline__ float join1(const half8& hi, const half8& lo, int e, int parts) {
    return parts == 2 ? (float)hi[e] + (float)lo[e] * H3_INV : (float)hi[e];
}

__global__ __launch_bounds__(256) void gather_h8_kernel(const float* __restrict__ box, int C, int Db, int Hb, int Wb,
                                                        int a0, int a1, int a2, float* __restrict__ dst, long pstride,
                                                        int G, int D, int H, int W, float scale, int parts) {
    const long v = (long)blockIdx.x * blockDim.x + threadIdx.x;
    const long V = (long)D * H * W;
    if (v >= V) return;
    const int z = (int)(v / ((long)H * W)), rem = (int)(v - (long)z * H * W);
    const int y = rem / W, x = rem - y * W;
    const int bz = ((a0 + z) % Db + Db) % Db, by = ((a1 + y) % Hb + Hb) % Hb, bx = ((a2 + x) % Wb + Wb) % Wb;
    const long bo = ((long)bz * Hb + by) * Wb + bx;
    const long bstride = (long)Db * Hb * Wb;
    for (int g = 0; parts * g < G; ++g) {
        half8 hi, lo;
#pragma unroll
        for (int e = 0; e < 8; ++e) {
            const int c = 8 * g + e;
            const float f = c < C ? box[c * bstride + bo] * scale : 0.f;
            hi[e] = (_Float16)f;
            lo[e] = (_Float16)((f - (float)hi[e]) * H3_SCALE);
        }
        *(half8*)(dst + ((long)(parts * g) * pstride + v) * 4) = hi;
        if (parts == 2) *(half8*)(dst + ((long)(2 * g + 1) * pstride + v) * 4) = lo;
    }
}

void launch_gather_h8(const float* box, int C, int Db, int Hb, int Wb, int a0, int a1, int a2,
                      float* dst, const Planes& geom, float scale, int parts, hipStream_t s) {
    const long V = geom.vox();
    hipLaunchKernelGGL(gather_h8_kernel, dim3((unsigned)((V + 255) / 256)), dim3(256), 0, s, box, C, Db, Hb, Wb,
                       a0, a1, a2, dst, geom.pstride, geom.G, geom.D, geom.H, geom.W, scale, parts);
}

__global__ __launch_bounds__(256) void from_planes_h8_kernel(const float* __restrict__ src, long pstride, long V, int C,
                                                             float* __restrict__ dst, int parts) {
    const long v = (long)blockIdx.x * blockDim.x + threadIdx.x;
    if (v >= V) return;
    for (int g = 0; 8 * g < C; ++g) {
        const half8 hi = ld8(src, parts * g, pstride, v);
        const half8 lo = parts == 2 ? ld8(src, 2 * g + 1, pstride, v) : hi;
#pragma unroll
        for (int e = 0; e < 8; ++e)
            if (8 * g + e < C) dst[(long)(8 * g + e) * V + v] = join1(hi, lo, e, parts);
    }
}

void launch_from_planes_h8(const float* src, const Planes& geom, int C, float* dst, int parts, hipStream_t s) {
    const long V = geom.vox();
    hipLaunchKernelGGL(from_planes_h8_kernel, dim3((unsigned)((V + 255) / 256)), dim3(256), 0, s, src, geom.pstride, V, C,
                       dst, parts);
}

template <typename OT>
__global__ __launch_bounds__(256) void head_h8_kernel(const float* __restrict__ y, const float* __restrict__ dy,
                                                      long ypstride, int D, int H, int W,
                                                      const float* __restrict__ xin, long xpstride, int XH, int XW,
                                                      int c0, int C, float k_disp, float k_dy, float k_x0,
                                                      OT* __restrict__ disp, OT* __restrict__ velo, int Db, int Hb,
                                                      int Wb, int a0, int a1, int a2, int parts, int pad,
                                                      int* __restrict__ bad) {
    const int Hi = H - 2 * pad, Wi = W - 2 * pad, c1 = pad > 0 ? pad : c0;
    const long vi = (long)blockIdx.x * blockDim.x + threadIdx.x;
    if (vi >= (long)D * Hi * Wi) return;
    const int z = (int)(vi / ((long)Hi * Wi)), rem = (int)(vi - (long)z * Hi * Wi);
// ... 48 lines not shown
```

### jax_nbody_emulator_with_dj_amd/csrc/nbe_kernels_head.h

```cpp
constexpr int HN4_ZB = 4;
constexpr int HN4_CT = 16, HN4_TAPU = 4 * HN4_CT;
constexpr int HN4_WG = 9 * HN4_TAPU;
constexpr int HN4_WC = 3 * HN4_WG;
constexpr int HN4_XBASE = 2 * HN4_WC;
constexpr int HN4_LDS_UNITS = HN4_XBASE + 2 * HQ_XB;

__global__ __launch_bounds__(512, 1) void conv_h3n4_kernel(ConvKArgs a) {
    constexpr int ZB = HN4_ZB, CT = HN4_CT, TAPU = HN4_TAPU, WG = HN4_WG, WC = HN4_WC, XBASE = HN4_XBASE, NT = 2, NW = 8;
    f32x4* lds = lds_h3;
    const half8* L8 = (const half8*)lds_h3;
    const int tid = threadIdx.x;
    const int lane = tid & 63;
    const int wave = __builtin_amdgcn_readfirstlane(tid >> 6);
    const int c = lane & 15, q = lane >> 4, kh = q & 1, ks = q >> 1;

    const int nzb = a.Dv / ZB;
    const int tile = xcd_tile(blockIdx.x, a.ntiles);
    const int zb = tile % nzb, tyx = tile / nzb;
    const int ty = tyx / a.tnx, tx = tyx - ty * a.tnx;
    const int y0 = ty * HP_ROWS, x0 = tx * HP_COLS, z0 = zb * ZB;
    const int nchunk = a.nchunk, nskip = a.nskip;
    const int nmain = nchunk * (ZB + 2), nstage = nmain + nskip * ZB;
    const long plane = (long)a.H * a.W * 16;
    const long to = (((long)z0 * a.H + y0) * a.W + x0) * 16;
// ... 53 lines not shown
    const int rowp = wave;
    const int aP = (ks * 4 + 2 * kh) * CT + c;
    const int bB = (2 * kh) * HQ_PP + rowp * HP_RS + c;
    const int bP1 = bB + ks, bP32 = bB + 32 * ks;
    constexpr int SH4 = HP_RS + 1, SH5 = HP_RS + 2, SH7 = 2 * HP_RS + 1;
    const half8 zero = {0, 0, 0, 0, 0, 0, 0, 0};

    auto group = [&](f32x4 (&Ym)[NT], f32x4 (&Yc)[NT], f32x4 (&Dm)[NT], f32x4 (&Dc)[NT], int wb, int xb) {
        auto pair = [&](int wa, int xp) {
            const half8 wh = L8[wa + aP], wl = L8[wa + CT + aP];
#pragma unroll
            for (int nt = 0; nt < NT; ++nt) {
                const half8 xh = L8[xp + 16 * nt], xl = L8[xp + HQ_PP + 16 * nt];
                const half8 dxh = L8[xp + HQ_XT + 16 * nt], dxl = L8[xp + HQ_XT + HQ_PP + 16 * nt];
                mm(Yc[nt], wh, xl); mm(Ym[nt], wh, xh); mm(Dm[nt], wh, dxh);
                mm(Dc[nt], wh, dxl); mm(Yc[nt], wl, xh); mm(Dc[nt], wl, dxh);
            }
            __builtin_amdgcn_sched_barrier(0);
        };
        pair(wb, xb + bP1);
        pair(wb + 2 * TAPU, xb + 2 + bP32);
        {
            const half8 a1w = L8[wb + 4 * TAPU + (2 * kh + ks) * CT + c];
            half8 a0 = L8[wb + 4 * TAPU + (2 * kh) * CT + c];
            a0 = ks ? a0 : zero;
            const int bS1 = xb + (2 * kh + 1 - ks) * HQ_PP + rowp * HP_RS + c + SH4;
#pragma unroll
            for (int nt = 0; nt < NT; ++nt) {
                const half8 b1x = L8[bS1 + 16 * nt], b1d = L8[bS1 + HQ_XT + 16 * nt];
                mm(Yc[nt], a1w, b1x); mm(Ym[nt], a0, b1x); mm(Dc[nt], a1w, b1d); mm(Dm[nt], a0, b1d);
            }
            __builtin_amdgcn_sched_barrier(0);
        }
        pair(wb + 5 * TAPU, xb + SH5 + bP32);
        pair(wb + 7 * TAPU, xb + SH7 + bP1);
    };
    auto skipgroup = [&](f32x4 (&Ym)[NT], f32x4 (&Yc)[NT], f32x4 (&Dm)[NT], f32x4 (&Dc)[NT], int wb, int xb) {
        const half8 a1w = L8[wb + (2 * kh + ks) * CT + c], a1d = L8[wb + 4 * CT + (2 * kh + ks) * CT + c];
        half8 a0 = L8[wb + (2 * kh) * CT + c], a0d = L8[wb + 4 * CT + (2 * kh) * CT + c];
        a0 = ks ? a0 : zero; a0d = ks ? a0d : zero;
        const int bS1 = xb + (2 * kh + 1 - ks) * HQ_PP + rowp * HP_RS + c + SH4;
        const bool nodx = a.flags & F_SKIP_NODX;
#pragma unroll
        for (int nt = 0; nt < NT; ++nt) {
            const half8 b1x = L8[bS1 + 16 * nt], b1d = L8[bS1 + HQ_XT + 16 * nt];
            mm(Yc[nt], a1w, b1x); mm(Ym[nt], a0, b1x);
            if (!nodx) { mm(Dc[nt], a1w, b1d); mm(Dm[nt], a0, b1d); }
            mm(Dc[nt], a1d, b1x); mm(Dm[nt], a0d, b1x);
        }
    };

    fetch(0);
    asm volatile("s_waitcnt vmcnt(0)" ::: "memory");
    __syncthreads();
    for (int chunk = 0; chunk < nchunk; ++chunk) {
        const int wb = (chunk & 1) * WC;
#pragma unroll
        for (int p = 0; p < ZB + 2; ++p) {
            const int s = chunk * (ZB + 2) + p;
            if (s + 1 < nstage) fetch(s + 1);
            const int xb = XBASE + (s & 1) * HQ_XB;
#pragma unroll
            for (int dz = 0; dz < 3; ++dz) {
                const int zo = p - dz;
                if (zo >= 0 && zo < ZB) group(ym[zo], yc[zo], dm[zo], dc[zo], wb + dz * WG, xb);
            }
            asm volatile("s_waitcnt vmcnt(0) lgkmcnt(0)" ::: "memory");
            __syncthreads();
        }
    }
    for (int sc = 0; sc < nskip; ++sc) {
        const int wb = ((nchunk + sc) & 1) * WC;
#pragma unroll
        for (int zo = 0; zo < ZB; ++zo) {
            const int s = nmain + sc * ZB + zo;
            if (s + 1 < nstage) fetch(s + 1);
            skipgroup(ym[zo], yc[zo], dm[zo], dc[zo], wb, XBASE + (s & 1) * HQ_XB);
            asm volatile("s_waitcnt vmcnt(0) lgkmcnt(0)" ::: "memory");
            __syncthreads();
        }
    }

    const bool act = a.flags & F_ACT, gauge = a.gout != nullptr;
    int unit = ks;
    const bool uok = unit < a.cout_groups;
    if (!uok) unit = a.cout_groups - 1;
    const f32x4 bv = *(const f32x4*)(a.bias + unit * 8 + 4 * kh);
    const f32x4 be = *(const f32x4*)(a.beta + unit * 8 + 4 * kh);
    f32x4 gv = {0.f, 0.f, 0.f, 0.f};
    if (gauge) gv = *(const f32x4*)(a.gout + unit * 8 + 4 * kh);
#pragma unroll
    for (int zo = 0; zo < ZB; ++zo) {
        const int z = z0 + zo;
#pragma unroll
        for (int nt = 0; nt < NT; ++nt) {
            const int yy = y0 + rowp, xx = x0 + 16 * nt + c;
            const bool ook = yy < a.Hv && xx < a.Wv;
            const long o = ook ? ((long)z * a.Ho + yy) * a.Wo + xx : 0;
            f32x4 v, dv;
#pragma unroll
            for (int e = 0; e < 4; ++e) {
                const float yp = ym[zo][nt][e] + yc[zo][nt][e] * H3_INV;
                v[e] = yp + bv[e];
                dv[e] = dm[zo][nt][e] + dc[zo][nt][e] * H3_INV + be[e] * yp;
            }
            if (act) {
#pragma unroll
                for (int e = 0; e < 4; ++e) {
                    dv[e] = v[e] > 0.f ? dv[e] : 0.01f * dv[e];
                    v[e] = v[e] >= 0.f ? v[e] : 0.01f * v[e];
                }
            }
            if (gauge) {
#pragma unroll
                for (int e = 0; e < 4; ++e) dv[e] += gv[e] * v[e];
            }
            if (uok && ook) {
                const long ob = ((long)(a.out_g0 + 2 * unit) * a.out_pstride + o) * 16 + 8 * kh;
                const long ol = ob + a.out_pstride * 16;
                half4 hi, lo;
                split4(v, hi, lo);
                *(half4*)((char*)a.y + ob) = hi;
                *(half4*)((char*)a.y + ol) = lo;
                split4(dv, hi, lo);
                *(half4*)((char*)a.dy + ob) = hi;
                *(half4*)((char*)a.dy + ol) = lo;
            }
        }
    }
}

static int launch_h3n4(ConvKArgs ka, int ctiles, hipStream_t s) {
    constexpr size_t smem = (size_t)HN4_LDS_UNITS * 16;
    static_assert(smem <= 160 * 1024, "LDS budget of one CU");
    if (ctiles != 1 || ka.cout_groups > 2 || (ka.flags & F_RES) || !ka.beta || ka.Dv % HN4_ZB != 0) return 1;
    if (ka.nchunk + ka.nskip > NBE_MAX_GROUPS) return 1;
    ensure_lds_limit((const void*)conv_h3n4_kernel, smem);
    ka.tny = (ka.Hv + HP_ROWS - 1) / HP_ROWS;
    ka.tnx = (ka.Wv + HP_COLS - 1) / HP_COLS;
    ka.ntiles = (ka.Dv / HN4_ZB) * ka.tny * ka.tnx;
    for (int chunk = 0; chunk < ka.nchunk; ++chunk) {
        const bool second = chunk >= ka.csplit;
        const long ps = second ? ka.in2_pstride : ka.in_pstride;
        const long off = (long)(second ? chunk - ka.csplit : chunk) * 4 * ps * 16;
        ka.gs[chunk] = {(const char*)(second ? ka.x2 : ka.x) + off, (const char*)(second ? ka.dx2 : ka.dx) + off,
                        (const char*)ka.w + (long)chunk * HN4_WC * 16, ps * 16};
    }
    for (int sc = 0; sc < ka.nskip; ++sc) {
        const bool second = sc >= ka.s_csplit;
        const long ps = second ? ka.s2_pstride : ka.s_pstride;
        const long off = (long)(second ? sc - ka.s_csplit : sc) * 4 * ps * 16;
        ka.gs[ka.nchunk + sc] = {(const char*)(second ? ka.xs2 : ka.xs) + off, (const char*)(second ? ka.dxs2 : ka.dxs) + off,
                                 (const char*)ka.ws + (long)sc * HN4_TAPU * 16, ps * 16};
    }
    ka.dws_delta = ka.nskip ? (const char*)ka.dws - (const char*)ka.ws : 0;
    hipLaunchKernelGGL(conv_h3n4_kernel, dim3(ka.ntiles), dim3(512), smem, s, ka);
    return 0;
}
```

### jax_nbody_emulator_with_dj_amd/csrc/nbe_kernels_internal.h

```cpp
#pragma once
#include "nbe_kernels.h"
#include <mutex>
#include <set>
#include <utility>

namespace nbe {

typedef float f32x4 __attribute__((ext_vector_type(4)));
typedef float f32x16 __attribute__((ext_vector_type(16)));
typedef _Float16 half8 __attribute__((ext_vector_type(8)));
typedef _Float16 half4 __attribute__((ext_vector_type(4)));

#define NBE_LDS_AS __attribute__((address_space(3)))
#define NBE_GLB_AS __attribute__((address_space(1)))

struct ConvGroupSrc { const char* x; const char* dx; const char* w; long psb; };

struct ConvKArgs {
    const float* x; const float* dx; long in_pstride;
    int D, H, W; long P; long in_off;
    int Dv, Hv, Wv; long Q;
    float* y; float* dy; long out_pstride; int out_g0;
    int Ho, Wo; int osz, oz, oy, ox;
    const float* r; const float* dr; long res_pstride;
    const float* bias; const float* w; const float* dw;
    int nchunk; int cout_groups; int flags; int ntiles;
    int tny, tnx;
    const float* gout;
    const float* beta;
    const float* x2; const float* dx2; long in2_pstride; int csplit;
    const float* xs; const float* dxs; long s_pstride; const float* xs2; const float* dxs2; long s2_pstride; int s_csplit;
    const float* ws; const float* dws; int nskip;
    long dws_delta;
    int up8; long set_stride;
    const float* wws; long wws_set_floats;
    const float* ww;
    const float* stem_w;
    ConvGroupSrc gs[NBE_MAX_GROUPS];
};

__device__ __forceinline__ void dma16(const float* src, f32x4* dst_wave_base) {
    __builtin_amdgcn_global_load_lds((const NBE_GLB_AS void*)src, (NBE_LDS_AS void*)dst_wave_base, 16, 0, 0);
}

inline void ensure_lds_limit(const void* kernel, size_t bytes) {
    static std::mutex mu;
    static std::set<std::pair<const void*, int>> done;
    int dev = 0;
    (void)hipGetDevice(&dev);
    std::lock_guard<std::mutex> lock(mu);
    if (done.insert({kernel, dev}).second)
        (void)hipFuncSetAttribute(kernel, hipFuncAttributeMaxDynamicSharedMemorySize, (int)bytes);
}

__device__ __forceinline__ int xcd_tile(int b, int nt) {
    const int qd = nt >> 3, rm = nt & 7, xcd = b & 7;
    return (xcd < rm ? xcd * (qd + 1) : rm * (qd + 1) + (xcd - rm) * qd) + (b >> 3);
}

int launch_conv_h3(const PackedW& pw, const ConvKArgs& ka, bool vel, bool has_dx, hipStream_t s);
void launch_pack_h3(const float* w_oidhw, int cout, int cin, int kind, const PackedW& pw, float* dst, hipStream_t s);
void launch_gather_h8(const float* box, int C, int Db, int Hb, int Wb, int a0, int a1, int a2,
                      float* dst, const Planes& geom, float scale, int parts, hipStream_t s);
void launch_from_planes_h8(const float* src, const Planes& geom, int C, float* dst, int parts, hipStream_t s);
void launch_head_h8(const Planes& y, const Planes& xin, int c0, int C, const HeadScale& hs, bool vel,
                    void* disp, void* velo, int out_dtype, int Db, int Hb, int Wb, int a0, int a1, int a2,
                    int parts, hipStream_t s, int pad = 0);

}
```

### jax_nbody_emulator_with_dj_amd/csrc/nbe_kernels_wino.h

```cpp

#ifndef NBE_EPI_MAX
#define NBE_EPI_MAX 1
#endif
#ifndef NBE_WINO_ZROW
#define NBE_WINO_ZROW 1
#endif
#ifndef NBE_WINO_ITEMREG
#define NBE_WINO_ITEMREG 1
#endif
#ifndef NBE_WINO_LOU
#define NBE_WINO_LOU (NBE_XF_F32 ? 0 : 1)
#endif
constexpr int NBE_MAX_WSTAGES = 32;
constexpr int NBE_MAX_WSKIP = 16;
constexpr float WINO_WSCALE = 16384.0f;
constexpr float WINO_WSCALE_F16 = 256.0f;

struct WinoSrc { const char* xa; const char* xb; long dxd; const char* w; long psb; float sb; int pad_; };

struct WinoKArgs {
    int H, W, Dv, Hv, Wv, Ho, Wo;
    int nchunk, cout_groups, flags, ntiles, tny, tnx;
    int zblock;
    float* y; float* dy; long out_pstride; int out_g0;
    const float* bias; const float* gout; const float* beta;
    const float* r; const float* dr; long res_pstride;
    float inv_scale;
    int nskip;
    long dws_delta;
    WinoSrc st[NBE_MAX_WSTAGES + NBE_MAX_WSKIP];
};

template <bool SKIP, bool NOVEL, bool F16 = false>
__global__ __launch_bounds__(512, 2) void conv_h3w_kernel(WinoKArgs a) {
    static_assert(!(F16 && NOVEL), "the float16 form has no displacement-only variant");
    typedef HGGeom<false> G;
    constexpr int NW = 8, CT = 64, TAPU = G::TAPU, WGU = G::WG, XBASE = G::XBASE, MT = 4, NT = 2, NTILE = 8;
    constexpr int ZROW = G::LDS_UNITS;
    f32x4* lds = lds_h3;
    const half8* L8 = (const half8*)lds_h3;
    half8* L8w = (half8*)lds_h3;
    const int tid = threadIdx.x;
    const int lane = tid & 63;
    const int wave = __builtin_amdgcn_readfirstlane(tid >> 6);
    const int c = lane & 15, q = lane >> 4, kh = q & 1, ks = q >> 1;

    const int nct = (a.cout_groups + 7) / 8;
    const int vt = xcd_tile(blockIdx.x, a.ntiles * nct);
    const int tile = vt / nct, ct = vt - tile * nct;
    const int npair = a.Dv >> 1;
    int zp, ty, tx;
    {
        const int zb = a.zblock;
        const int full = (npair / zb) * zb;
        const int per_blk = zb * a.tny * a.tnx;
        if (tile < (npair / zb) * per_blk) {
            const int blk = tile / per_blk, r = tile - blk * per_blk;
            const int zi = r % zb, tyx = r / zb;
            zp = blk * zb + zi; ty = tyx / a.tnx; tx = tyx - ty * a.tnx;
        } else {
            const int r = tile - (npair / zb) * per_blk, rem = npair - full;
            const int zi = r % rem, tyx = r / rem;
            zp = full + zi; ty = tyx / a.tnx; tx = tyx - ty * a.tnx;
        }
    }
    const int y0 = ty * (NOVEL ? 2 * HP_ROWS : HP_ROWS), x0 = tx * HP_COLS, z0 = 2 * zp;
    const int nst = 4 * a.nchunk;

    const long to = (((long)z0 * a.H + y0) * a.W + x0) * 16;
    const long wcm = (long)ct * nst * WGU * 16, wcs = (long)ct * a.nskip * TAPU * 16;

    struct Nxt { const char *xa, *xb, *w0; long dxd, psb; float sb; } nx;
    auto set_next = [&](int s) {
        const WinoSrc e = a.st[s];
        nx.xa = e.xa + to; nx.xb = e.xb + to; nx.dxd = e.dxd; nx.psb = e.psb; nx.w0 = e.w + (SKIP && s >= nst ? wcs : wcm); nx.sb = e.sb;
    };
    unsigned lane16 = (unsigned)lane << 4;
    asm volatile("" : "+v"(lane16));
    auto dma_w = [&](int buf, int t) {
        const int n = wave + NW * t;
        unsigned l16 = (unsigned)lane;
        if (NBE_WINO_ZROW && !F16) l16 = lane16;
        else asm volatile("v_lshlrev_b32 %0, 4, %0" : "+v"(l16));
        if (n < G::NWI) dma16s(nx.w0 + (long)n * 1024, l16, lds + buf * WGU + n * 64);
    };
    auto dma_raw = [&](int buf) {
        unsigned l16 = (unsigned)lane;
        asm volatile("v_lshlrev_b32 %0, 4, %0" : "+v"(l16));
        dma16s(nx.w0 + (wave < 4 ? 0 : a.dws_delta) + (long)(wave & 3) * 1024, l16, lds + buf * WGU + wave * 64);
#pragma unroll
        for (int t = 0; t < 6; ++t) {
            const int tensor = t / 3, n = wave + NW * (t % 3), pl = n / 6, k = n - 6 * pl;
            const int u = k * 64 + lane;
            const int uu = u < HP_PL ? u : HP_PL - 1;
            const int row = (uu * 241) >> 13, col = uu - row * HP_RS;
            if (u < HP_PL)
                dma16s(nx.xa + (tensor ? nx.dxd : 0) + (long)pl * nx.psb, (unsigned)(row * a.W + col) * 16u,
                       lds + XBASE + buf * HQ_XB + tensor * HQ_XT + pl * HQ_PP + k * 64);
        }
    };
    constexpr bool ITEMREG = NBE_WINO_ITEMREG && !F16;
    int it_uu[3] = {0, 0, 0};
    unsigned it_go[3] = {0u, 0u, 0u};
    if (ITEMREG) {
#pragma unroll
        for (int j = 0; j < 3; ++j) {
            const int u = ((wave + NW * j) % 6) * 64 + lane;
            it_uu[j] = u < HP_PL ? u : HP_PL - 1;
            const int row = (it_uu[j] * 241) >> 13, col = it_uu[j] - row * HP_RS;
            it_go[j] = (unsigned)(row * a.W + col) * 16u;
        }
#pragma unroll
        for (int j = 0; j < 3; ++j) asm volatile("" : "+v"(it_uu[j]), "+v"(it_go[j]));
    }
    auto item_unit = [&](int j, bool& valid) {
        if (ITEMREG) {
            valid = lane < HP_PL - ((wave + NW * j) % 6) * 64;
// ... 202 lines not shown
        preXl(); preW();
        NBE_SB; MM8(Y, wl, xh, -1, nb, px); NBE_SB;
        preXh();
        NBE_SB; MM8(DY, wl, dxh, -1, nb, px); NBE_SB;
    };

    constexpr int SH4 = HP_RS + 1, SH5 = HP_RS + 2, SH7 = 2 * HP_RS + 1;
    auto stage = [&](f32x4 (&Y)[NTILE], f32x4 (&DY)[NTILE], int s, auto nxt) {
        constexpr int NXT = decltype(nxt)::value;
        constexpr bool px = NXT == 1;
        const bool pre = px && s + 1 != 2 * a.nchunk;
        if (NXT) set_next(s + 1);
        int par = s & 1;
        asm volatile("" : "+s"(par));
        int nb = 1 - par;
        asm volatile("" : "+s"(nb));
        const int wb = par * WGU, xb = XBASE + par * HQ_XB;
        const int wbn = nb * WGU, xbn = XBASE + nb * HQ_XB;
        Stg g;
        Xf xf;
        auto hk = [&](int k) { xf_step(g, xf, k); };
        auto none = [] {};
        if (NXT == 2) dma_raw(nb);
        if (px) st_load(0, g);
        pair(Y, DY, 0, nb, px, wb, xb + bP1,
             [&] { LB(xl, xb + 2 + bP32 + HQ_PP); }, [&] { LA(wh, wb + 2 * TAPU + aP); }, [&] { LB(xh, xb + 2 + bP32); },
             none, false, nohook, none);
        half8 a1[MT], a2[MT], b1x[NT], b1d[NT];
        const int aS = wb + 4 * TAPU + (2 * kh + (F16 ? ks : 0)) * CT + c;
        const int bS = xb + (2 * kh + ks) * HQ_PP + rowp * HP_RS + c + SH4;
        pair(Y, DY, -1, nb, px, wb + 2 * TAPU, xb + 2 + bP32,
             [&] { LB(b1x, bS); }, [&] { LA(a1, aS); }, [&] { LB(b1d, bS + HQ_XT); }, none,
             px, hk, [&] { if (px) { st_write(0, nb, xf); st_load(1, g); } });
        const half8 zero = {0, 0, 0, 0, 0, 0, 0, 0};
        if (F16) {
            NBE_SB; MM8(Y, a1, b1x, -1, 0, false); NBE_SB;
            LB(xl, xb + SH5 + bP32 + HQ_PP); LB(xh, xb + SH5 + bP32); LA(wh, wb + 5 * TAPU + aP);
            NBE_SB; MM8(DY, a1, b1d, -1, 0, false); NBE_SB;
        } else {
#if NBE_WINO_LOU
        NBE_SB; MM8(Y, a1, b1x, -1, 0, false); NBE_SB;
#else
        {
            const _Float16 m1 = ks ? kInv : (_Float16)1.0f;
#pragma unroll
            for (int mt = 0; mt < MT; ++mt) a1[mt] = a1[mt] * m1;
        }
        NBE_SB; MM8(Y, a1, b1x, -1, 0, false, true); NBE_SB;
#endif
#if NBE_WINO_ZROW
        LA(a2, ks ? ZROW + c : aS + CT);
#else
        LA(a2, aS + CT);
#endif
        LB(xl, xb + SH5 + bP32 + HQ_PP);
        NBE_SB; MM8(DY, a1, b1d, -1, 0, false); NBE_SB;
        LB(xh, xb + SH5 + bP32); LA(wh, wb + 5 * TAPU + aP);
#if NBE_WINO_ZROW
        NBE_SB; MM8(Y, a2, b1x, -1, 0, false); NBE_SB;
#else
#pragma unroll
        for (int mt = 0; mt < MT; ++mt) a2[mt] = ks ? zero : a2[mt];
        NBE_SB; MM8(Y, a2, b1x, -1, 0, false, true); NBE_SB;
#endif
        MM8(DY, a2, b1d, -1, 0, false); NBE_SB;
        }
        pair(Y, DY, -1, nb, px, wb + 5 * TAPU, xb + SH5 + bP32,
             [&] { LB(xl, xb + SH7 + bP1 + HQ_PP); }, [&] { LA(wh, wb + 7 * TAPU + aP); }, [&] { LB(xh, xb + SH7 + bP1); },
             none, px, hk, [&] { if (px) { st_write(1, nb, xf); st_load(2, g); } });
        pair(Y, DY, -1, nb, px, wb + 7 * TAPU, xb + SH7 + bP1,
             [&] { if (pre) LB(xl, xbn + bP1 + HQ_PP); }, [&] { if (pre) LA(wh, wbn + aP); }, [&] { if (pre) LB(xh, xbn + bP1); },
             [&] { asm volatile("s_waitcnt vmcnt(0) lgkmcnt(0)\n\ts_barrier" ::: "memory"); },
             px, hk, [&] { if (px) st_write(2, nb, xf); });
    };

    auto raw_stage = [&](f32x4 (&Y)[NTILE], f32x4 (&DY)[NTILE], int s, bool px) {
        if (px) set_next(s + 1);
        int par = s & 1;
        asm volatile("" : "+s"(par));
        int nb = 1 - par;
        asm volatile("" : "+s"(nb));
        const int wb = par * WGU, xb = XBASE + par * HQ_XB;
        if (px) dma_raw(nb);
        half8 a1[MT], a2[MT], d1[MT], d2[MT], bx[NT], bd[NT];
        const half8 zero = {0, 0, 0, 0, 0, 0, 0, 0};
        const _Float16 m1 = ks ? kInv : (_Float16)1.0f;
        const int aS = wb + (2 * kh) * CT + c;
        const int bS = xb + (2 * kh + ks) * HQ_PP + rowp * HP_RS + c + SH4;
        if (F16) {
            const int aF = wb + (2 * kh + ks) * CT + c;
            LA(a1, aF); LB(bx, bS); LB(bd, bS + HQ_XT); LA(d1, aF + TAPU);
            NBE_SB; MM8(Y, a1, bx, -1, 0, false); NBE_SB;
            MM8(DY, a1, bd, -1, 0, false); NBE_SB;
            MM8(DY, d1, bx, -1, 0, false); NBE_SB;
            asm volatile("s_waitcnt vmcnt(0) lgkmcnt(0)\n\ts_barrier" ::: "memory");
            return;
        }
        LA(a1, aS); LB(bx, bS); LA(a2, aS + CT); LB(bd, bS + HQ_XT);
#pragma unroll
        for (int mt = 0; mt < MT; ++mt) a1[mt] = a1[mt] * m1;
        NBE_SB; MM8(Y, a1, bx, -1, 0, false, true); NBE_SB;
        if (!NOVEL) LA(d1, aS + TAPU);
#pragma unroll
        for (int mt = 0; mt < MT; ++mt) a2[mt] = ks ? zero : a2[mt];
        NBE_SB; MM8(Y, a2, bx, -1, 0, false, true); NBE_SB;
        if (!NOVEL) LA(d2, aS + TAPU + CT);
        if (NOVEL || !(a.flags & F_SKIP_NODX)) {
            NBE_SB; MM8(DY, a1, bd, -1, 0, false); NBE_SB;
            MM8(DY, a2, bd, -1, 0, false); NBE_SB;
        }
        if (!NOVEL) {
#pragma unroll
            for (int mt = 0; mt < MT; ++mt) { d1[mt] = d1[mt] * m1; d2[mt] = ks ? zero : d2[mt]; }
            NBE_SB; MM8(DY, d1, bx, -1, 0, false, true); NBE_SB;
            MM8(DY, d2, bx, -1, 0, false, true); NBE_SB;
        }
        asm volatile("s_waitcnt vmcnt(0) lgkmcnt(0)\n\ts_barrier" ::: "memory");
    };

    {
        if (NBE_WINO_ZROW && !F16 && tid < 64) L8w[ZROW + tid] = half8{0, 0, 0, 0, 0, 0, 0, 0};
        set_next(0);
#pragma unroll
        for (int k = 0; k < G::NWS; ++k) dma_w(0, k);
        {
            Stg g0, g1, g2;
            st_load(0, g0); st_load(1, g1); st_load(2, g2);
            st_store(0, 0, g0); st_store(1, 0, g1); st_store(2, 0, g2);
        }
        asm volatile("s_waitcnt vmcnt(0) lgkmcnt(0)" ::: "memory");
        __syncthreads();
        LA(wh, aP); LB(xl, XBASE + bP1 + HQ_PP); LB(xh, XBASE + bP1);
    }

    auto butterfly = [&] {
            asm volatile("s_nop 15\n\ts_nop 15" ::: "memory");
#pragma unroll
            for (int t = 0; t < NTILE; ++t) {
                f32x4 p, m;
#pragma unroll
                for (int e = 0; e < 4; ++e) { p[e] = acc_read(YA[t][e]); m[e] = acc_read(YB[t][e]); }
                YA[t] = p + m; YB[t] = p - m;
                asm volatile("" : "+a"(YA[t]), "+a"(YB[t]));
                __builtin_amdgcn_sched_barrier(0);
#pragma unroll
                for (int e = 0; e < 4; ++e) { p[e] = acc_read(DA[t][e]); m[e] = acc_read(DB[t][e]); }
                DA[t] = p + m; DB[t] = p - m;
                asm volatile("" : "+a"(DA[t]), "+a"(DB[t]));
                __builtin_amdgcn_sched_barrier(0);
            }
            asm volatile("s_nop 7" ::: "memory");
            LA(wh, aP); LB(xl, XBASE + bP1 + HQ_PP); LB(xh, XBASE + bP1);
    };
    const int npairs = 2 * a.nchunk;
    for (int s2 = 0; s2 + 1 < npairs; ++s2) {
        if (s2 == a.nchunk) butterfly();
        stage(YA, DA, 2 * s2, std::integral_constant<int, 1>());
        stage(YB, DB, 2 * s2 + 1, std::integral_constant<int, 1>());
    }
    if (npairs - 1 == a.nchunk) butterfly();
    stage(YA, DA, 2 * npairs - 2, std::integral_constant<int, 1>());
    stage(YB, DB, 2 * npairs - 1, std::integral_constant<int, SKIP ? 2 : 0>());
    if (SKIP) {
        for (int sc = 0; sc < a.nskip; ++sc) {
            raw_stage(YA, DA, nst + 2 * sc, true);
            raw_stage(YB, DB, nst + 2 * sc + 1, sc + 1 < a.nskip);
        }
    }
#undef NBE_SB
#undef SNAKE
    asm volatile("s_nop 15\n\ts_nop 15" ::: "memory");

    const bool act = a.flags & F_ACT, gauge = !NOVEL && a.gout != nullptr;
    f32x4 bv[MT], be[MT], gv[MT];
    int unit[MT];
    bool uok[MT];
#pragma unroll
    for (int mt = 0; mt < MT; ++mt) {
        unit[mt] = ct * (CT / 8) + 2 * mt + ks;
        uok[mt] = unit[mt] < a.cout_groups;
        if (!uok[mt]) unit[mt] = a.cout_groups - 1;
        bv[mt] = *(const f32x4*)(a.bias + unit[mt] * 8 + 4 * kh);
        be[mt] = f32x4{0.f, 0.f, 0.f, 0.f};
        if (!NOVEL) be[mt] = *(const f32x4*)(a.beta + unit[mt] * 8 + 4 * kh);
        gv[mt] = f32x4{0.f, 0.f, 0.f, 0.f};
        if (!NOVEL && gauge) gv[mt] = *(const f32x4*)(a.gout + unit[mt] * 8 + 4 * kh);
    }
#pragma unroll
    for (int mt = 0; mt < MT; ++mt) asm volatile("" : "+v"(bv[mt]), "+v"(be[mt]), "+v"(gv[mt]));
    long ob_mt[MT];
#pragma unroll
    for (int mt = 0; mt < MT; ++mt) ob_mt[mt] = (long)(a.out_g0 + (F16 ? 1 : 2) * unit[mt]) * a.out_pstride * 16 + 8 * kh;
    const long ol_off = a.out_pstride * 16;
    auto epilogue = [&](f32x4 (&Y)[NTILE], f32x4 (&DY)[NTILE], int z) {
        int o[NT];
        bool ook[NT], ook2[NT];
#pragma unroll
        for (int nt = 0; nt < NT; ++nt) {
            const int yy = y0 + rowp, xx = x0 + 16 * nt + c;
            ook[nt] = yy < a.Hv && xx < a.Wv;
            ook2[nt] = NOVEL && yy + HP_ROWS < a.Hv && xx < a.Wv;
            o[nt] = ook[nt] ? (z * a.Ho + yy) * a.Wo + xx : z * a.Ho * a.Wo;
        }
        half4 r0[F16 ? NTILE : 1], r1[F16 ? NTILE : 1];
        const bool res = F16 && (a.flags & F_RES);
        if (F16 && res) {
#pragma unroll
            for (int t = 0; t < NTILE; ++t) {
                const int mt = t / NT, nt = t % NT;
                const long rb = ((long)unit[mt] * a.res_pstride + (long)o[nt]) * 16 + 8 * kh;
                r0[t] = *(const half4*)((const char*)a.r + rb);
                r1[t] = *(const half4*)((const char*)a.dr + rb);
            }
#pragma unroll
            for (int t = 0; t < NTILE; ++t) asm volatile("" : "+v"(r0[t]), "+v"(r1[t]));
        }
#pragma unroll
        for (int mt = 0; mt < MT; ++mt) {
#pragma unroll
            for (int nt = 0; nt < NT; ++nt) {
                const int t = mt * NT + nt;
                f32x4 v, dv;
                __builtin_amdgcn_sched_barrier(0);
#pragma unroll
                for (int e = 0; e < 4; ++e) {
                    const float yp = acc_read(Y[t][e]) * a.inv_scale;
                    v[e] = yp + bv[mt][e];
                    dv[e] = acc_read(DY[t][e]) * a.inv_scale + be[mt][e] * yp;
                }
                if (F16 && res) {
#pragma unroll
                    for (int e = 0; e < 4; ++e) { v[e] += (float)r0[t][e]; dv[e] += (float)r1[t][e]; }
                }
                if (act) {
#pragma unroll
                    for (int e = 0; e < 4; ++e) {
                        dv[e] = v[e] > 0.f ? dv[e] : 0.01f * dv[e];
                        v[e] = (F16 || !NBE_EPI_MAX) ? (v[e] >= 0.f ? v[e] : 0.01f * v[e]) : __builtin_fmaxf(v[e], 0.01f * v[e]);
                    }
                }
                if (gauge) {
#pragma unroll
                    for (int e = 0; e < 4; ++e) dv[e] += gv[mt][e] * v[e];
                }
                if (F16) {
                    if (uok[mt] && ook[nt]) {
                        const long ob = ob_mt[mt] + (long)o[nt] * 16;
                        half4 h, dh;
#pragma unroll
                        for (int e = 0; e < 4; ++e) { h[e] = (_Float16)v[e]; dh[e] = (_Float16)dv[e]; }
                        *(half4*)((char*)a.y + ob) = h;
                        *(half4*)((char*)a.dy + ob) = dh;
                    }
                } else
                if (NOVEL) {
#pragma unroll
                    for (int e = 0; e < 4; ++e) {
                        dv[e] = acc_read(DY[t][e]) * a.inv_scale + bv[mt][e];
                        if (act) dv[e] = dv[e] >= 0.f ? dv[e] : 0.01f * dv[e];
                    }
                    const long ob = ob_mt[mt] + (long)o[nt] * 16;
                    const long ol = ob + ol_off;
                    const long r8 = (long)HP_ROWS * a.Wo * 16;
                    half4 hi, lo;
                    if (uok[mt] && ook[nt]) {
                        split4(v, hi, lo);
                        *(half4*)((char*)a.y + ob) = hi;
                        *(half4*)((char*)a.y + ol) = lo;
                    }
                    if (uok[mt] && ook2[nt]) {
                        split4(dv, hi, lo);
                        *(half4*)((char*)a.y + ob + r8) = hi;
                        *(half4*)((char*)a.y + ol + r8) = lo;
                    }
                } else
                if (uok[mt] && ook[nt]) {
                    const long ob = ob_mt[mt] + (long)o[nt] * 16;
                    const long ol = ob + ol_off;
                    half4 hi, lo;
                    split4(v, hi, lo);
                    *(half4*)((char*)a.y + ob) = hi;
                    *(half4*)((char*)a.y + ol) = lo;
                    split4(dv, hi, lo);
                    *(half4*)((char*)a.dy + ob) = hi;
                    *(half4*)((char*)a.dy + ol) = lo;
                }
            }
        }
    };
    epilogue(YA, DA, z0);
    epilogue(YB, DB, z0 + 1);
}

__global__ __launch_bounds__(256) void pack_h3w_kernel(const float* __restrict__ w, int cout, int cin, int nchunk, long total,
                                                       _Float16* __restrict__ dst, int* __restrict__ flag, int f16) {
    const long idx = (long)blockIdx.x * blockDim.x + threadIdx.x;
    if (idx >= total) return;
    long r = idx;
    const int j = (int)(r % 8); r /= 8;
    const int co = (int)(r % 64); r /= 64;
    const int u = (int)(r % 4); r /= 4;
    const int tap = (int)(r % 9); r /= 9;
    const int stage = (int)(r % (4 * nchunk)); r /= 4 * nchunk;
    const int ct = (int)r;
    const int chunk = stage >> 2, xi = stage & 3;
    const int h = u >> 1, part = u & 1;
    const int ci = f16 ? chunk * 32 + 8 * u + j : chunk * 16 + 8 * h + j, oc = ct * 64 + co;
    float v = 0.f;
    if (oc < cout && ci < cin) {
        const float* p = w + (((size_t)oc * cin + ci) * 3) * 9 + tap;
        const float w0 = p[0], w1 = p[9], w2 = p[18];
        v = xi == 0 ? w0 : xi == 1 ? 0.5f * (w0 + w1 + w2) : xi == 2 ? 0.5f * (w0 - w1 + w2) : -w2;
    }
    v *= f16 ? WINO_WSCALE_F16 : WINO_WSCALE;
    if (!(fabsf(v) <= 60000.f)) { atomicOr(flag, 1); v = 0.f; }
    const _Float16 hi = (_Float16)v;
    dst[idx] = (part == 0 || f16) ? hi : (_Float16)(v - (float)hi);
}

void launch_pack_h3w(const float* w_oidhw, int cout, int cin, int cin_pad, int ctiles, float* dst, int* flag, hipStream_t s, int prec) {
    const bool f16 = prec == PREC_F16;
    const int nchunk = cin_pad / (f16 ? 32 : 16);
    const long total = (long)ctiles * 4 * nchunk * 9 * 4 * 64 * 8;
    hipLaunchKernelGGL(pack_h3w_kernel, dim3((unsigned)((total + 255) / 256)), dim3(256), 0, s, w_oidhw, cout, cin, nchunk, total,
                       (_Float16*)dst, flag, f16 ? 1 : 0);
}

static int launch_h3w(const ConvKArgs& ka_in, const float* ww, const float* wws, long wws_set_floats, int ctiles, hipStream_t s,
                      bool novel = false, bool f16 = false) {
    typedef HGGeom<false> G;
    constexpr size_t smem = (size_t)(G::LDS_UNITS + 64) * 16;
    static_assert(smem <= 160 * 1024, "LDS budget of one CU");
    ConvKArgs ka = ka_in;
    if (f16) {
        if (novel || (ka.nchunk & 1) || (ka.csplit < ka.nchunk && (ka.csplit & 1))) return 1;
        if (ka.nskip > 0 && ((ka.nskip & 1) || (ka.s_csplit < ka.nskip && (ka.s_csplit & 1)) || (ka.flags & F_SKIP_NODX))) return 1;
        ka.nchunk /= 2; if (ka.csplit < (1 << 29)) ka.csplit /= 2;
        ka.nskip /= 2; if (ka.s_csplit < (1 << 29)) ka.s_csplit /= 2;
    }
    if (!ww || (!f16 && (ka.flags & F_RES)) || (ka.Dv & 1) || 4 * ka.nchunk > NBE_MAX_WSTAGES || (!novel && !ka.beta)) return 1;
    if (ka.nskip > 0 && (!wws || 2 * ka.nskip > NBE_MAX_WSKIP)) return 1;
    if (ctiles != (ka.cout_groups + 7) / 8) return 1;
    if (std::max(ka.in_pstride, ka.csplit < ka.nchunk ? ka.in2_pstride : 0L) * 16 + 16L * (HP_ROWS + 2) * ka.W >= (1L << 32) - (1L << 20)) return 1;
    WinoKArgs wa;
    wa.H = ka.H; wa.W = ka.W; wa.Dv = ka.Dv; wa.Hv = ka.Hv; wa.Wv = ka.Wv; wa.Ho = ka.Ho; wa.Wo = ka.Wo;
    wa.nchunk = ka.nchunk; wa.cout_groups = ka.cout_groups; wa.flags = ka.flags;
    const int trows = novel ? 2 * HP_ROWS : HP_ROWS;
    wa.tny = (ka.Hv + trows - 1) / trows;
    wa.tnx = (ka.Wv + HP_COLS - 1) / HP_COLS;
    wa.ntiles = (ka.Dv / 2) * wa.tny * wa.tnx;
    wa.y = ka.y; wa.dy = ka.dy; wa.out_pstride = ka.out_pstride; wa.out_g0 = ka.out_g0;
    wa.bias = ka.bias; wa.gout = novel ? nullptr : ka.gout; wa.beta = novel ? nullptr : ka.beta;
    const long rows8 = (long)HP_ROWS * ka.W * 16;
    wa.inv_scale = 1.0f / (f16 ? WINO_WSCALE_F16 : WINO_WSCALE);
    wa.r = ka.r; wa.dr = ka.dr; wa.res_pstride = ka.res_pstride;
    wa.zblock = std::min(8, ka.Dv / 2);
    wa.nskip = ka.nskip; wa.dws_delta = wws_set_floats * 4;
    static const int XI[2][2] = {{1, 2}, {0, 3}};
    static const int PA[4] = {0, 1, 2, 1}, PB[4] = {2, 2, 1, 3};
    static const float SB[4] = {-1.f, 1.f, -1.f, -1.f};
    const long plane = (long)ka.H * ka.W * 16;
    for (int ph = 0; ph < 2; ++ph)
        for (int chunk = 0; chunk < ka.nchunk; ++chunk)
            for (int ab = 0; ab < 2; ++ab) {
                const int xi = XI[ph][ab];
                const bool second = chunk >= ka.csplit;
                const long ps = second ? ka.in2_pstride : ka.in_pstride;
                const char* x = (const char*)(second ? ka.x2 : ka.x);
                const char* dx = (const char*)(second ? ka.dx2 : ka.dx);
                const long off = (long)(second ? chunk - ka.csplit : chunk) * 4 * ps * 16;
                WinoSrc& e = wa.st[(ph * ka.nchunk + chunk) * 2 + ab];
                e.xa = x + off + PA[xi] * plane; e.xb = x + off + PB[xi] * plane; e.dxd = novel ? rows8 : dx - x;
                e.w = (const char*)ww + (long)(chunk * 4 + xi) * G::WG * 16; e.psb = ps * 16; e.sb = SB[xi]; e.pad_ = 0;
            }
    for (int sc = 0; sc < ka.nskip; ++sc)
        for (int ab = 0; ab < 2; ++ab) {
            const bool second = sc >= ka.s_csplit;
            const long ps = second ? ka.s2_pstride : ka.s_pstride;
            const char* x = (const char*)(second ? ka.xs2 : ka.xs);
            const char* dx = (const char*)(second ? ka.dxs2 : ka.dxs);
            const long off = (long)(second ? sc - ka.s_csplit : sc) * 4 * ps * 16 + ab * plane;
            WinoSrc& e = wa.st[4 * ka.nchunk + 2 * sc + ab];
            e.xa = x + off; e.xb = e.xa; e.dxd = novel ? rows8 : dx - x; e.w = (const char*)wws + (long)sc * G::TAPU * 16; e.psb = ps * 16; e.sb = 0.f; e.pad_ = 0;
        }
    const bool skip = ka.nskip > 0;
    if (novel) wa.dws_delta = 0;
    auto kern = f16 ? (skip ? conv_h3w_kernel<true, false, true> : conv_h3w_kernel<false, false, true>)
              : novel ? (skip ? conv_h3w_kernel<true, true> : conv_h3w_kernel<false, true>)
              : (skip ? conv_h3w_kernel<true, false> : conv_h3w_kernel<false, false>);
    ensure_lds_limit((const void*)kern, smem);
    dim3 grid(wa.ntiles * ctiles, 1, 1), block(512, 1, 1);
    hipLaunchKernelGGL(kern, grid, block, smem, s, wa);
    return 0;
}
```

Measured before the change: 97.28 million.

## Fuse next block's 1x1 skip conv into conv_r00 epilogue as head-skip residual

```diff
diff --git a/jax_nbody_emulator_with_dj_amd/csrc/nbe_engine.cpp b/jax_nbody_emulator_with_dj_amd/csrc/nbe_engine.cpp
--- a/jax_nbody_emulator_with_dj_amd/csrc/nbe_engine.cpp
+++ b/jax_nbody_emulator_with_dj_amd/csrc/nbe_engine.cpp
@@ -176,6 +176,7 @@
     int64_t plan_logged = 0;
     int* gauge_flag = nullptr;
     int* wino_flag = nullptr; bool wino_ok = false;
+    float* headskip_w = nullptr; bool headskip_ok = false;
     float act_scale = 1.f;
     float bias_scale = 1.f;
     bool bias_dirty = true;
@@ -448,6 +449,7 @@
 
 static bool wino_f16_layer(int prec, bool vel, int cin_pad) { return prec == PREC_F16 && vel && cin_pad % 32 == 0 && cin_pad / 32 <= 8; }
 static bool wino_env_off() { return getenv("NBE_WINO") && atoi(getenv("NBE_WINO")) == 0; }
+static bool headskip_env_off() { return getenv("NBE_HEADSKIP") && atoi(getenv("NBE_HEADSKIP")) == 0; }
 static bool up8_launch(const nbe_ctx* c, const Layer& L, bool has_dx) { return prec_is_half(c->prec) && (!c->vel || has_dx) && L.pw.cin_pad <= 64; }
 
 static int run_conv(nbe_ctx* c, const Layer& L, const ConvLaunch& cl_in, bool has_dx) {
@@ -456,17 +458,20 @@
     const bool g6 = c->gauge_active && L.g6 && has_dx;
     const bool nov = !c->vel && c->prec == PREC_F16X3 && L.kind == 0 && L.pw.ww && c->wino_ok;
     if (c->gauge_active) { cl.gout = L.gout; cl.beta = g6 ? L.beta : nullptr; }
-    if (cl.skw) {
+    if (cl.skw || cl.hs_res.x) {
         if (!((g6 || nov) && c->fuse && L.fskip)) return fail("internal error: fused skip requested for %s/%s", L.block.c_str(), L.layer.c_str());
         cl.bias = L.bias_f;
     }
     const PackedW& pw = (g6 && L.kind == 0 && L.pwn.w) ? L.pwn : L.pw;
     cl.wino = (g6 || nov) && c->wino_ok && &pw == &L.pw && pw.ww && (!cl.skw || cl.skw->ww) && (c->prec == PREC_F16 || !(cl.flags & F_RES)) &&
               (cl.Dv & 1) == 0 && cl.in_off == 0 && cl.osz == 1 && !wino_env_off();
+    if (cl.hs_out.x && !(cl.wino && cl.skw)) return fail("internal error: %s/%s cannot write the next block's skip", L.block.c_str(), L.layer.c_str());
     int pe = -1; hipEvent_t ea = nullptr, eb = nullptr;
     if (c->prof) {
         std::string pn = cl.wino ? std::string(c->prec == PREC_F16 ? "conv_h1w<FLAT3,vel,dx>" : c->vel ? "conv_h3w<FLAT3,vel,dx>" : "conv_h3w<FLAT3,novel>")
                                  : conv_name(pw, c->vel, has_dx, g6, cl.set < 0);
+        if (cl.hs_out.x) pn.insert(pn.size() - 1, ",headskip");
+        if (cl.hs_res.x) pn.insert(pn.size() - 1, ",res");
         static const bool per_layer = getenv("NBE_PROF_LAYERS") && atoi(getenv("NBE_PROF_LAYERS")) == 1;
         if (per_layer) pn += " " + L.block + "/" + L.layer;
         pe = prof_entry(c, pn);
@@ -501,6 +506,20 @@
     return c->fuse && L1->fskip != nullptr && (!wino_only_fuse(c) || (!wino_env_off() && (nres & 1) == 0));
 }
 
+static bool head_skip_pair(const nbe_ctx* c, const Tensor& hq, int nq, int ny) {
+    const auto lq = c->layers.find("conv_r00/conv_1"), ly = c->layers.find("conv_r01/conv_1");
+    if (lq == c->layers.end() || ly == c->layers.end()) return false;
+    return c->headskip_ok && !headskip_env_off() && !wino_env_off() && c->prec == PREC_F16X3 && c->vel && c->gauge_active && c->wino_ok &&
+           block_fused(c, &lq->second, nq) && block_fused(c, &ly->second, ny) && (nq & 1) == 0 && ny % 4 == 0 &&
+           h3w_offsets_fit(hq.p.pstride, hq.p.W);
+}
+static Tensor alloc_head_skip(nbe_ctx* c, const Tensor& q) {
+    Tensor t;
+    t.p = ws_planes(c, 1, q.p.D, q.p.H, q.p.W, &t.off);
+    t.pad = q.pad;
+    return t;
+}
+
 static Tensor alloc_hidden(nbe_ctx* c, int cmid, int nz, const Tensor& x, bool fused) {
     const int pad = x.pad, sy = pad ? 0 : 2;
     if (fused && !pad) return talloc(c, cmid, nz, x.p.H, x.p.W);
@@ -508,13 +527,15 @@
 }
 
 static int resblock_part(nbe_ctx* c, const char* name, const Tensor& x, const Tensor& h, const Tensor& s,
-                         int js, int ns, int jh, int nh, bool has_dx, bool final_act, const int* zr, const Tensor* x2 = nullptr) {
+                         int js, int ns, int jh, int nh, bool has_dx, bool final_act, const int* zr, const Tensor* x2 = nullptr,
+                         const Tensor* hs_out = nullptr, const Tensor* hs_in = nullptr) {
     const Layer *Ls = find_layer(c, name, "skip"), *L0 = find_layer(c, name, "conv_0"), *L1 = find_layer(c, name, "conv_1");
     if (!Ls || !L0 || !L1) return fail("missing layers of block %s", name);
     const int H = x.p.H, W = x.p.W, pad = x.pad;
     const bool fused = block_fused(c, L1, ns);
     if (fused && (h.p.H != H || h.p.W != W)) return fail("internal: hidden tensor of fused block %s lacks the input's pitch", name);
     if (x2 && (!fused || x2->p.H != H || x2->p.W != W || x2->pad != pad)) return fail("internal: two-source input of block %s", name);
+    if ((hs_out || hs_in) && !fused) return fail("internal: head-skip residual on unfused block %s", name);
     const Tensor sv = zview(s, js, ns), hv = zview(h, jh, nh);
     const Tensor xs = zview(x, js, ns + 4);
     const int64_t sk_off = (2L * H + (pad ? pad : 2)) * W + (pad ? pad : 2);
@@ -535,9 +556,11 @@
     fill_halo(c, hv);
     {
         ConvLaunch cl; cl.in = zview(h, js, ns + 2).p; cl.Dv = ns; cl.Hv = s.p.H - 2 * pad; cl.Wv = s.p.W - 2 * pad; cl.out = inner(sv);
-        if (fused) { cl.sk = xs.p; cl.sk_off = sk_off; cl.skw = L1->pwn.w ? &Ls->pwn : &Ls->pw; cl.flags = (final_act ? F_ACT : 0) | (has_dx ? 0 : F_SKIP_NODX);
+        if (fused && hs_in) { cl.hs_res = zview(*hs_in, js, ns + 4).p; cl.hs_off = sk_off; cl.flags = final_act ? F_ACT : 0; }
+        else if (fused) { cl.sk = xs.p; cl.sk_off = sk_off; cl.skw = L1->pwn.w ? &Ls->pwn : &Ls->pw; cl.flags = (final_act ? F_ACT : 0) | (has_dx ? 0 : F_SKIP_NODX);
                      if (x2) { cl.sk2 = zview(*x2, js, ns + 4).p; cl.sk_split_ch = c->mid; } }
         else { cl.res = inner(sv); cl.flags = F_RES | (final_act ? F_ACT : 0); }
+        if (hs_out) { cl.hs_out = inner(zview(*hs_out, js, ns)); cl.hs_w = c->headskip_w; }
         if (run_conv(c, *L1, cl, true)) return 1;
         org_conv(x, 2, og); og[0] += js;
         if (final_act) probe_act(c, *L1, cl.out, 0, og, cl.Dv, cl.Hv, cl.Wv, pad != 0, zr);
@@ -546,7 +569,8 @@
     return 0;
 }
 
-static int resblock(nbe_ctx* c, const char* name, const Tensor& x, bool has_dx, bool final_act, int cout, int cmid, Tensor* out) {
+static int resblock(nbe_ctx* c, const char* name, const Tensor& x, bool has_dx, bool final_act, int cout, int cmid, Tensor* out,
+                    Tensor* hs_out = nullptr, const Tensor* hs_in = nullptr) {
     const Layer* L1 = find_layer(c, name, "conv_1");
     if (!L1) return fail("missing layers of block %s", name);
     const int D = x.p.D, pad = x.pad;
@@ -554,7 +578,11 @@
     Tensor s = tallocp(c, cout, D - 4, x.p.H - 2 * pad - 2 * sy, x.p.W - 2 * pad - 2 * sy, pad);
     Tensor h = alloc_hidden(c, cmid, D - 2, x, block_fused(c, L1, D - 4));
     if (s.off < 0 || h.off < 0) return fail("workspace exhausted in block %s", name);
-    if (resblock_part(c, name, x, h, s, 0, D - 4, 0, D - 2, has_dx, final_act, nullptr)) return 1;
+    if (hs_out && head_skip_pair(c, h, D - 4, D - 8)) {
+        *hs_out = alloc_head_skip(c, s);
+        if (hs_out->off < 0) return fail("workspace exhausted in block %s", name);
+    } else hs_out = nullptr;
+    if (resblock_part(c, name, x, h, s, 0, D - 4, 0, D - 2, has_dx, final_act, nullptr, nullptr, hs_out, hs_in)) return 1;
     tfree(c, h);
     int og[3];
     org_conv(x, 2, og);
@@ -931,11 +959,12 @@
 
     if (upblock(c, "up_r0", r, cat0)) return 1;
     tfree(c, r);
-    if (resblock(c, "conv_r00", cat0, true, true, m, 2 * m, &r)) return 1;
+    Tensor rs;
+    if (resblock(c, "conv_r00", cat0, true, true, m, 2 * m, &r, &rs)) return 1;
     tfree(c, cat0);
 
-    if (resblock(c, "conv_r01", r, true, false, c->out_chan, m, yout)) return 1;
-    tfree(c, r);
+    if (resblock(c, "conv_r01", r, true, false, c->out_chan, m, yout, nullptr, rs.off >= 0 ? &rs : nullptr)) return 1;
+    tfree(c, r); tfree(c, rs);
     return 0;
 }
 
@@ -1041,10 +1070,19 @@
     Tensor q = tallocp(c, m, S + 4, Hs - 2 * sy, Ws - 2 * sy, pad), hy = alloc_hidden(c, m, S + 2, q, block_fused(c, Lr01, S));
     Tensor y = tallocp(c, c->out_chan, S, Hs - 4 * sy, Ws - 4 * sy, pad);
     if (cat.off < 0 || hq.off < 0 || q.off < 0 || hy.off < 0 || y.off < 0) return fail("workspace exhausted (level-0 decoder slabs)");
-    for (int z = 0, n = 0; z < Yo; z += n) {
-        n = std::min(S, Yo - z);
+    auto slab_planes = [&](int z) {
+        int n = std::min(S, Yo - z);
         if (c->pipe.active && c->pipe.out_async && Yo - z > PIPE_EDGE && Yo - z - n < PIPE_EDGE)
             n = Yo - z - PIPE_EDGE;
+        return n;
+    };
+    bool hs = true;
+    for (int z = 0, n = 0; z < Yo && hs; z += n) { n = slab_planes(z); hs = head_skip_pair(c, hq, z == 0 ? n + 4 : n, n); }
+    Tensor qs;
+    if (hs) { qs = alloc_head_skip(c, q); if (qs.off < 0) return fail("workspace exhausted (level-0 decoder slabs)"); }
+    const Tensor* qsp = hs ? &qs : nullptr;
+    for (int z = 0, n = 0; z < Yo; z += n) {
+        n = slab_planes(z);
         const bool first = z == 0;
         const int c0 = first ? 0 : 8, cn = first ? n + 8 : n;
         set_org(cat, skip0.org[0] + z, skip0.org[1], skip0.org[2]);
@@ -1055,16 +1093,17 @@
         const Tensor sk = two ? zview(skip0, z, std::min(S + 8, skip0.p.D - z)) : cat;
         const Tensor* up2 = two ? &cat : nullptr;
         if (first) {
-            if (resblock_part(c, "conv_r00", sk, hq, q, 0, n + 4, 0, n + 6, true, true, nullptr, up2)) return 1;
-            if (resblock_part(c, "conv_r01", q, hy, y, 0, n, 0, n + 2, true, false, nullptr)) return 1;
+            if (resblock_part(c, "conv_r00", sk, hq, q, 0, n + 4, 0, n + 6, true, true, nullptr, up2, qsp)) return 1;
+            if (resblock_part(c, "conv_r01", q, hy, y, 0, n, 0, n + 2, true, false, nullptr, nullptr, nullptr, qsp)) return 1;
         } else {
-            if (resblock_part(c, "conv_r00", sk, hq, q, 4, n, 6, n, true, true, nullptr, up2)) return 1;
-            if (resblock_part(c, "conv_r01", q, hy, y, 0, n, 2, n, true, false, nullptr)) return 1;
+            if (resblock_part(c, "conv_r00", sk, hq, q, 4, n, 6, n, true, true, nullptr, up2, qsp)) return 1;
+            if (resblock_part(c, "conv_r01", q, hy, y, 0, n, 2, n, true, false, nullptr, nullptr, nullptr, qsp)) return 1;
         }
         if (z + n < Yo) {
             carry_planes(c, cat, n, 0, 8);
             carry_planes(c, hq, n, 0, 6);
             carry_planes(c, q, n, 0, 4);
+            if (hs) carry_planes(c, qs, n, 0, 4);
             carry_planes(c, hy, n, 0, 2);
         }
         run_head(c, zview(y, 0, n), zview(tin, z, n + 96), ho, z);
@@ -1073,7 +1112,7 @@
             c->prog->post(c->pipe.active && c->pipe.out_async ? c->down_stream : c->stream,
                           c->prog_k * 1000 + (int)(1000L * (z + n) / Yo), c->prog_n * 1000);
     }
-    tfree(c, cat); tfree(c, hq); tfree(c, q); tfree(c, hy); tfree(c, y);
+    tfree(c, cat); tfree(c, hq); tfree(c, q); tfree(c, hy); tfree(c, y); tfree(c, qs);
     tfree(c, r); tfree(c, skip0);
     return 0;
 }
@@ -1195,7 +1234,7 @@
     const int geo[18] = {Db, Hb, Wb, o0, o1, o2, D, H, W, out_dtype, OD, OH, OW, a0, a1, a2, c->slab, c->prec};
     memcpy(k.geo, geo, sizeof geo);
     k.f[0] = Dz; k.f[1] = vel_fac; k.f[2] = c->act_scale;
-    k.epoch = c->epoch; k.flags = (c->pyx ? 1 : 0) | (c->pz ? 2 : 0) | (c->gauge_active ? 4 : 0) | (c->fuse ? 8 : 0) | (wino_env_off() ? 16 : 0);
+    k.epoch = c->epoch; k.flags = (c->pyx ? 1 : 0) | (c->pz ? 2 : 0) | (c->gauge_active ? 4 : 0) | (c->fuse ? 8 : 0) | (wino_env_off() ? 16 : 0) | (headskip_env_off() ? 32 : 0);
     nbe_ctx::GraphVal& g = c->graphs[k];
     g.used = ++c->graph_clock;
     if (!g.exec && g.seen++ == 0) {
@@ -1289,10 +1328,23 @@
             if (c->vel) launch_pack_h3w_skip(c->prec == PREC_F16 ? L.dwn_f : L.dwn, L.cout, L.cin, L.pw, L.pw.ww + L.pw.floats, c->wino_flag, c->stream);
         }
     }
+    c->headskip_ok = false;
+    {
+        auto ls = c->layers.find("conv_r01/skip"), lq = c->layers.find("conv_r00/conv_1");
+        if (ls != c->layers.end() && lq != c->layers.end() && c->prec == PREC_F16X3 && c->vel && c->gauge_active && c->fuse) {
+            const Layer &Ls = ls->second, &Lq = lq->second;
+            if (Ls.b_sub && Ls.pwn.dw && Ls.cout <= 4 && Ls.cin <= 64 && Lq.pw.ww && Lq.pw.ctiles == 1 && Lq.cout == Ls.cin) {
+                if (!c->headskip_w) HIPCHK(hipMalloc((void**)&c->headskip_w, HEADSKIP_W_FLOATS * 4));
+                launch_pack_headskip(Ls.wn, Ls.dwn, Ls.cout, Ls.cin, c->headskip_w, c->wino_flag, c->stream);
+                c->headskip_ok = true;
+            }
+        }
+    }
     int bad = 0;
     HIPCHK(hipMemcpyAsync(&bad, c->wino_flag, 4, hipMemcpyDeviceToHost, c->stream));
     HIPCHK(hipStreamSynchronize(c->stream));
-    c->wino_ok = bad == 0;
+    c->wino_ok = (bad & 1) == 0;
+    c->headskip_ok = c->headskip_ok && (bad & 2) == 0;
     if (!c->vel) c->fuse = c->novel_fuse && c->wino_ok;
     if (c->prec == PREC_F16) c->fuse = c->fuse && c->wino_ok;
     return 0;
@@ -1599,7 +1651,7 @@
     prof_collect(c);
     free_layers(c);
     (void)hipFree(c->probe.bits); (void)hipFree(c->probe.count);
-    (void)hipFree(c->ws); (void)hipFree(c->box_in); (void)hipFree(c->box_out); (void)hipFree(c->gauge_flag); (void)hipFree(c->wino_flag); (void)hipFree(c->flags);
+    (void)hipFree(c->ws); (void)hipFree(c->box_in); (void)hipFree(c->box_out); (void)hipFree(c->gauge_flag); (void)hipFree(c->wino_flag); (void)hipFree(c->headskip_w); (void)hipFree(c->flags);
     drop_graphs(c);
     if (c->ev_g0) (void)hipEventDestroy(c->ev_g0);
     if (c->ev_g1) (void)hipEventDestroy(c->ev_g1);
diff --git a/jax_nbody_emulator_with_dj_amd/csrc/nbe_kernels.h b/jax_nbody_emulator_with_dj_amd/csrc/nbe_kernels.h
--- a/jax_nbody_emulator_with_dj_amd/csrc/nbe_kernels.h
+++ b/jax_nbody_emulator_with_dj_amd/csrc/nbe_kernels.h
@@ -66,6 +66,10 @@
     int64_t sk_off = 0;
     const PackedW* skw = nullptr;
     bool wino = false;
+    Planes hs_out;
+    const float* hs_w = nullptr;
+    Planes hs_res;
+    int64_t hs_off = 0;
 };
 
 int launch_conv(const PackedW& pw, const ConvLaunch& L, bool vel, bool has_dx, hipStream_t s);
@@ -81,6 +85,9 @@
 void launch_pack_h3w(const float* w_oidhw, int cout, int cin, int cin_pad, int ctiles, float* dst, int* flag, hipStream_t s,
                      int prec = PREC_F16X3);
 void launch_pack_h3w_skip(const float* w_oidhw, int cout, int cin, const PackedW& pw, float* dst, int* flag, hipStream_t s);
+constexpr int HEADSKIP_W_FLOATS = 2 * 6 * 64 * 4;
+void launch_pack_headskip(const float* w_oidhw, const float* dw_oidhw, int cout, int cin, float* dst, int* flag, hipStream_t s);
+bool h3w_offsets_fit(int64_t in_pstride, int W);
 
 void launch_gather(const float* box, int C, int Db, int Hb, int Wb, int a0, int a1, int a2,
                    const Planes& dst, float scale, int prec, hipStream_t s);
diff --git a/jax_nbody_emulator_with_dj_amd/csrc/nbe_kernels.hip b/jax_nbody_emulator_with_dj_amd/csrc/nbe_kernels.hip
--- a/jax_nbody_emulator_with_dj_amd/csrc/nbe_kernels.hip
+++ b/jax_nbody_emulator_with_dj_amd/csrc/nbe_kernels.hip
@@ -242,6 +242,11 @@
         if (L.sk_split_ch > 0) { ka.xs2 = L.sk2.x + o; ka.dxs2 = L.sk2.dx + o; ka.s2_pstride = L.sk2.pstride; ka.s_csplit = L.sk_split_ch / 16; }
         ka.ws = L.skw->w; ka.dws = L.skw->dw; ka.nskip = L.skw->cin_pad / 16;
     }
+    ka.hs_w = L.hs_w; ka.hs_y = L.hs_out.x; ka.hs_dy = L.hs_out.dx;
+    ka.hs_r = L.hs_res.x ? L.hs_res.x + L.hs_off * 4 : nullptr; ka.hs_dr = L.hs_res.x ? L.hs_res.dx + L.hs_off * 4 : nullptr;
+    if (ka.hs_y && (!ka.hs_w || !ka.hs_dy || L.hs_out.H != L.out.H || L.hs_out.W != L.out.W)) return 1;
+    if (ka.hs_r && (!ka.hs_dr || L.hs_res.H != L.in.H || L.hs_res.W != L.in.W)) return 1;
+    if ((ka.hs_y || ka.hs_r) && pw.prec != PREC_F16X3) return 1;
     ka.ntiles = (int)((ka.Q + TILE_VOX - 1) / TILE_VOX);
     if (prec_is_half(pw.prec)) return launch_conv_h3(pw, ka, vel, has_dx, s);
     const int ct = pw.ctiles;
diff --git a/jax_nbody_emulator_with_dj_amd/csrc/nbe_kernels_h3.hip b/jax_nbody_emulator_with_dj_amd/csrc/nbe_kernels_h3.hip
--- a/jax_nbody_emulator_with_dj_amd/csrc/nbe_kernels_h3.hip
+++ b/jax_nbody_emulator_with_dj_amd/csrc/nbe_kernels_h3.hip
@@ -1798,6 +1798,11 @@
         !(ka.flags & F_RES) && ka.nskip == 0 && !ka.beta) {
         if (split) return vel ? launch_stem<true>(ka, s) : launch_stem<false>(ka, s);
         return vel ? launch_stem<true, false>(ka, s) : launch_stem<false, false>(ka, s);
+    }
+    if (ka.hs_y || ka.hs_r) {
+        if (!(split && vel && has_dx && ka.beta && pw.mode == MODE_FLAT3 && ka.in_off == 0 && ka.osz == 1)) return 1;
+        if (ka.hs_r) return (ka.hs_y || pw.cout_t != 16 || ka.nskip != 0) ? 1 : launch_h3n4(ka, ct, s);
+        return (pw.cout_t == 16 || !ka.ww || ka.nskip == 0) ? 1 : launch_h3w(ka, ka.ww, ka.wws, ka.wws_set_floats, ct, s);
     }
     if ((ka.nskip > 0 || ka.csplit < ka.nchunk) && !(ka.beta && split)) {
         if (split && !vel && ka.ww && pw.mode == MODE_FLAT3 && ka.in_off == 0 && ka.osz == 1)
@@ -1892,6 +1897,24 @@
                        1, pw.mode, pw.cin_pad / 16, halves, 1, 2, pw.cout_t, (_Float16*)dst, 16384.0f, flag);
 }
 
+__global__ __launch_bounds__(256) void pack_headskip_kernel(const float* __restrict__ w, const float* __restrict__ dw, int cout, int cin,
+                                                            _Float16* __restrict__ dst, int* __restrict__ flag) {
+    const int idx = blockIdx.x * blockDim.x + threadIdx.x;
+    if (idx >= HEADSKIP_W_FLOATS * 2) return;
+    const int j = idx & 7, lane = (idx >> 3) & 63, k = (idx >> 9) % 6, mp = idx / (6 * 512);
+    const int m = lane & 15, q = lane >> 4, ch = 16 * (2 * mp + (j >> 2)) + 4 * q + (j & 3);
+    float v = 0.f;
+    if (m < cout && ch < cin) v = (k < 3 ? w : dw)[(size_t)m * cin + ch] * WINO_WSCALE;
+    if (!(fabsf(v) <= 60000.f)) { atomicOr(flag, 2); v = 0.f; }
+    const _Float16 hi = (_Float16)v;
+    dst[idx] = k % 3 == 0 ? hi : k % 3 == 1 ? (_Float16)((float)hi * H3_INV) : (_Float16)(v - (float)hi);
+}
+
+void launch_pack_headskip(const float* w_oidhw, const float* dw_oidhw, int cout, int cin, float* dst, int* flag, hipStream_t s) {
+    hipLaunchKernelGGL(pack_headskip_kernel, dim3(HEADSKIP_W_FLOATS * 2 / 256), dim3(256), 0, s, w_oidhw, dw_oidhw, cout, cin,
+                       (_Float16*)dst, flag);
+}
+
 void launch_pack_h3(const float* w_oidhw, int cout, int cin, int kind, const PackedW& pw, float* dst, hipStream_t s) {
     if (pw.stem && kind == 0 && (dst == pw.w || dst == pw.dw)) {
         const int parts = pw.prec == PREC_F16X3 ? 2 : 1;
diff --git a/jax_nbody_emulator_with_dj_amd/csrc/nbe_kernels_head.h b/jax_nbody_emulator_with_dj_amd/csrc/nbe_kernels_head.h
--- a/jax_nbody_emulator_with_dj_amd/csrc/nbe_kernels_head.h
+++ b/jax_nbody_emulator_with_dj_amd/csrc/nbe_kernels_head.h
@@ -159,6 +159,19 @@
     }
 
     const bool act = a.flags & F_ACT, gauge = a.gout != nullptr;
+    const bool res = a.hs_r != nullptr && q == 0;
+    auto res_off = [&](int zo, int nt) {
+        const int yy = y0 + rowp, xx = x0 + 16 * nt + c;
+        return yy < a.Hv && xx < a.Wv ? (((long)(z0 + zo) * a.H + yy) * a.W + xx) * 4 : -1L;
+    };
+    const f32x4 zero4 = {0.f, 0.f, 0.f, 0.f};
+    f32x4 rn[NT], drn[NT];
+#pragma unroll
+    for (int nt = 0; nt < NT; ++nt) {
+        const long ro = res ? res_off(0, nt) : -1L;
+        rn[nt] = ro >= 0 ? *(const f32x4*)(a.hs_r + ro) : zero4;
+        drn[nt] = ro >= 0 ? *(const f32x4*)(a.hs_dr + ro) : zero4;
+    }
     int unit = ks;
     const bool uok = unit < a.cout_groups;
     if (!uok) unit = a.cout_groups - 1;
@@ -169,6 +182,14 @@
 #pragma unroll
     for (int zo = 0; zo < ZB; ++zo) {
         const int z = z0 + zo;
+        f32x4 rc[NT], drc[NT];
+#pragma unroll
+        for (int nt = 0; nt < NT; ++nt) {
+            rc[nt] = rn[nt]; drc[nt] = drn[nt];
+            const long ro = res && zo + 1 < ZB ? res_off(zo + 1, nt) : -1L;
+            rn[nt] = ro >= 0 ? *(const f32x4*)(a.hs_r + ro) : zero4;
+            drn[nt] = ro >= 0 ? *(const f32x4*)(a.hs_dr + ro) : zero4;
+        }
 #pragma unroll
         for (int nt = 0; nt < NT; ++nt) {
             const int yy = y0 + rowp, xx = x0 + 16 * nt + c;
@@ -177,9 +198,9 @@
             f32x4 v, dv;
 #pragma unroll
             for (int e = 0; e < 4; ++e) {
-                const float yp = ym[zo][nt][e] + yc[zo][nt][e] * H3_INV;
+                const float yp = ym[zo][nt][e] + yc[zo][nt][e] * H3_INV + rc[nt][e];
                 v[e] = yp + bv[e];
-                dv[e] = dm[zo][nt][e] + dc[zo][nt][e] * H3_INV + be[e] * yp;
+                dv[e] = dm[zo][nt][e] + dc[zo][nt][e] * H3_INV + drc[nt][e] + be[e] * yp;
             }
             if (act) {
 #pragma unroll
@@ -211,6 +232,7 @@
     constexpr size_t smem = (size_t)HN4_LDS_UNITS * 16;
     static_assert(smem <= 160 * 1024, "LDS budget of one CU");
     if (ctiles != 1 || ka.cout_groups > 2 || (ka.flags & F_RES) || !ka.beta || ka.Dv % HN4_ZB != 0) return 1;
+    if (ka.hs_r && (ka.nskip != 0 || ka.cout_groups != 1)) return 1;
     if (ka.nchunk + ka.nskip > NBE_MAX_GROUPS) return 1;
     ensure_lds_limit((const void*)conv_h3n4_kernel, smem);
     ka.tny = (ka.Hv + HP_ROWS - 1) / HP_ROWS;
diff --git a/jax_nbody_emulator_with_dj_amd/csrc/nbe_kernels_internal.h b/jax_nbody_emulator_with_dj_amd/csrc/nbe_kernels_internal.h
--- a/jax_nbody_emulator_with_dj_amd/csrc/nbe_kernels_internal.h
+++ b/jax_nbody_emulator_with_dj_amd/csrc/nbe_kernels_internal.h
@@ -36,6 +36,8 @@
     const float* wws; long wws_set_floats;
     const float* ww;
     const float* stem_w;
+    const float* hs_w; float* hs_y; float* hs_dy;
+    const float* hs_r; const float* hs_dr;
     ConvGroupSrc gs[NBE_MAX_GROUPS];
 };
 
diff --git a/jax_nbody_emulator_with_dj_amd/csrc/nbe_kernels_wino.h b/jax_nbody_emulator_with_dj_amd/csrc/nbe_kernels_wino.h
--- a/jax_nbody_emulator_with_dj_amd/csrc/nbe_kernels_wino.h
+++ b/jax_nbody_emulator_with_dj_amd/csrc/nbe_kernels_wino.h
@@ -28,11 +28,17 @@
     float inv_scale;
     int nskip;
     long dws_delta;
+    int headskip;
+    const char* hsw;
+    float* hs_y; float* hs_dy;
     WinoSrc st[NBE_MAX_WSTAGES + NBE_MAX_WSKIP];
 };
 
+static_assert(HEADSKIP_W_FLOATS == 2 * 6 * 64 * 4, "the packer and the kernel agree on the operand block");
+constexpr int HS_UNITS = 2 * 6 * 64;
 template <bool SKIP, bool NOVEL, bool F16 = false>
 __global__ __launch_bounds__(512, 2) void conv_h3w_kernel(WinoKArgs a) {
+    constexpr bool HSK = SKIP && !NOVEL && !F16;
     static_assert(!(F16 && NOVEL), "the float16 form has no displacement-only variant");
     typedef HGGeom<false> G;
     constexpr int NW = 8, CT = 64, TAPU = G::TAPU, WGU = G::WG, XBASE = G::XBASE, MT = 4, NT = 2, NTILE = 8;
@@ -401,6 +407,12 @@
         asm volatile("" : "+s"(nb));
         const int wb = par * WGU, xb = XBASE + par * HQ_XB;
         if (px) dma_raw(nb);
+        if (HSK && !px && a.headskip) {
+            unsigned l16 = (unsigned)lane;
+            asm volatile("v_lshlrev_b32 %0, 4, %0" : "+v"(l16));
+            dma16s(a.hsw + (long)wave * 1024, l16, lds + wave * 64);
+            if (wave < HS_UNITS / 64 - NW) dma16s(a.hsw + (long)(wave + NW) * 1024, l16, lds + (wave + NW) * 64);
+        }
         half8 a1[MT], a2[MT], d1[MT], d2[MT], bx[NT], bd[NT];
         const half8 zero = {0, 0, 0, 0, 0, 0, 0, 0};
         const _Float16 m1 = ks ? kInv : (_Float16)1.0f;
@@ -511,7 +523,8 @@
 #pragma unroll
     for (int mt = 0; mt < MT; ++mt) ob_mt[mt] = (long)(a.out_g0 + (F16 ? 1 : 2) * unit[mt]) * a.out_pstride * 16 + 8 * kh;
     const long ol_off = a.out_pstride * 16;
-    auto epilogue = [&](f32x4 (&Y)[NTILE], f32x4 (&DY)[NTILE], int z) {
+    auto epilogue = [&](f32x4 (&Y)[NTILE], f32x4 (&DY)[NTILE], int z, auto hs) {
+        constexpr bool HS = decltype(hs)::value;
         int o[NT];
         bool ook[NT], ook2[NT];
 #pragma unroll
@@ -534,10 +547,15 @@
 #pragma unroll
             for (int t = 0; t < NTILE; ++t) asm volatile("" : "+v"(r0[t]), "+v"(r1[t]));
         }
-#pragma unroll
-        for (int mt = 0; mt < MT; ++mt) {
-#pragma unroll
-            for (int nt = 0; nt < NT; ++nt) {
+        f32x4 sy, sd;
+        half4 qh[2], ql[2], dqh[2], dql[2];
+        auto mmv = [&](f32x4& acc, const half8& A, const half8& B) {
+            asm("s_nop 1\n\tv_mfma_f32_16x16x32_f16 %0, %1, %2, %0" : "+v"(acc) : "v"(A), "v"(B));
+        };
+#pragma unroll
+        for (int i = 0; i < NTILE; ++i) {
+            {
+                const int mt = HS ? i % MT : i / NT, nt = HS ? i / MT : i % NT;
                 const int t = mt * NT + nt;
                 f32x4 v, dv;
                 __builtin_amdgcn_sched_barrier(0);
@@ -593,6 +611,36 @@
                         *(half4*)((char*)a.y + ol + r8) = lo;
                     }
                 } else
+                if (HS) {
+                    const int h = mt & 1;
+                    const long ob = ob_mt[mt] + (long)o[nt] * 16;
+                    const long ol = ob + ol_off;
+                    split4(v, qh[h], ql[h]);
+                    split4(dv, dqh[h], dql[h]);
+                    if (uok[mt] && ook[nt]) {
+                        *(half4*)((char*)a.y + ob) = qh[h];
+                        *(half4*)((char*)a.y + ol) = ql[h];
+                        *(half4*)((char*)a.dy + ob) = dqh[h];
+                        *(half4*)((char*)a.dy + ol) = dql[h];
+                    }
+                    if (h) {
+                        auto cat = [](const half4& p, const half4& r) { return __builtin_shufflevector(p, r, 0, 1, 2, 3, 4, 5, 6, 7); };
+                        const half8 bh = cat(qh[0], qh[1]), bl = cat(ql[0], ql[1]), dh = cat(dqh[0], dqh[1]), dl = cat(dql[0], dql[1]);
+                        const int wa = (mt >> 1) * 6 * 64 + lane;
+                        if (mt == 1) { sy = f32x4{0.f, 0.f, 0.f, 0.f}; sd = sy; }
+                        half8 w0 = L8[wa], w1 = L8[wa + 64], w2 = L8[wa + 128];
+                        mmv(sy, w0, bh); mmv(sd, w0, dh); mmv(sy, w1, bl); mmv(sd, w1, dl); mmv(sy, w2, bh); mmv(sd, w2, dh);
+                        w0 = L8[wa + 192]; w1 = L8[wa + 256]; w2 = L8[wa + 320];
+                        mmv(sd, w0, bh); mmv(sd, w1, bl); mmv(sd, w2, bh);
+                    }
+                    if (mt == MT - 1) {
+                        asm volatile("s_nop 15\n\ts_nop 3" : "+v"(sy), "+v"(sd));
+                        if (q == 0 && ook[nt]) {
+                            *(f32x4*)(a.hs_y + (long)o[nt] * 4) = sy * a.inv_scale;
+                            *(f32x4*)(a.hs_dy + (long)o[nt] * 4) = sd * a.inv_scale;
+                        }
+                    }
+                } else
                 if (uok[mt] && ook[nt]) {
                     const long ob = ob_mt[mt] + (long)o[nt] * 16;
                     const long ol = ob + ol_off;
@@ -607,8 +655,15 @@
             }
         }
     };
-    epilogue(YA, DA, z0);
-    epilogue(YB, DB, z0 + 1);
+    if constexpr (HSK) {
+        if (a.headskip) {
+            epilogue(YA, DA, z0, std::true_type());
+            epilogue(YB, DB, z0 + 1, std::true_type());
+            return;
+        }
+    }
+    epilogue(YA, DA, z0, std::false_type());
+    epilogue(YB, DB, z0 + 1, std::false_type());
 }
 
 __global__ __launch_bounds__(256) void pack_h3w_kernel(const float* __restrict__ w, int cout, int cin, int nchunk, long total,
@@ -645,6 +700,8 @@
                        (_Float16*)dst, flag, f16 ? 1 : 0);
 }
 
+bool h3w_offsets_fit(int64_t in_pstride, int W) { return in_pstride * 16 + 16L * (HP_ROWS + 2) * W < (1L << 32) - (1L << 20); }
+
 static int launch_h3w(const ConvKArgs& ka_in, const float* ww, const float* wws, long wws_set_floats, int ctiles, hipStream_t s,
                       bool novel = false, bool f16 = false) {
     typedef HGGeom<false> G;
@@ -660,7 +717,8 @@
     if (!ww || (!f16 && (ka.flags & F_RES)) || (ka.Dv & 1) || 4 * ka.nchunk > NBE_MAX_WSTAGES || (!novel && !ka.beta)) return 1;
     if (ka.nskip > 0 && (!wws || 2 * ka.nskip > NBE_MAX_WSKIP)) return 1;
     if (ctiles != (ka.cout_groups + 7) / 8) return 1;
-    if (std::max(ka.in_pstride, ka.csplit < ka.nchunk ? ka.in2_pstride : 0L) * 16 + 16L * (HP_ROWS + 2) * ka.W >= (1L << 32) - (1L << 20)) return 1;
+    if (!h3w_offsets_fit(std::max(ka.in_pstride, ka.csplit < ka.nchunk ? ka.in2_pstride : 0L), ka.W)) return 1;
+    if (ka.hs_y && (novel || f16 || ka.nskip == 0 || ctiles != 1)) return 1;
     WinoKArgs wa;
     wa.H = ka.H; wa.W = ka.W; wa.Dv = ka.Dv; wa.Hv = ka.Hv; wa.Wv = ka.Wv; wa.Ho = ka.Ho; wa.Wo = ka.Wo;
     wa.nchunk = ka.nchunk; wa.cout_groups = ka.cout_groups; wa.flags = ka.flags;
@@ -675,6 +733,7 @@
     wa.r = ka.r; wa.dr = ka.dr; wa.res_pstride = ka.res_pstride;
     wa.zblock = std::min(8, ka.Dv / 2);
     wa.nskip = ka.nskip; wa.dws_delta = wws_set_floats * 4;
+    wa.headskip = ka.hs_y != nullptr; wa.hsw = (const char*)ka.hs_w; wa.hs_y = ka.hs_y; wa.hs_dy = ka.hs_dy;
     static const int XI[2][2] = {{1, 2}, {0, 3}};
     static const int PA[4] = {0, 1, 2, 1}, PB[4] = {2, 2, 1, 3};
     static const float SB[4] = {-1.f, 1.f, -1.f, -1.f};
```

Result: no change. 97.99 million (median of 6 runs) (+0.7%).
